# Improbable-AI/walk-these-ways

Hardware: AMD Instinct MI355X
Metric: env-steps/sec (sim+PPO) (higher is better)
Workload: dtype f32

## Files before the change

include/go1ppo.h:

```cpp
#ifndef GO1PPO_H
#define GO1PPO_H
#include <stdint.h>

#ifdef __cplusplus
extern "C" {
#endif

#define GO1PPO_ABI_VERSION 3
#define GO1PPO_MAX_ACTIONS 32

int go1ppo_elu_fwd(void* y, int64_t rows, int cols, int ld, const void* lat, int lat_ld, int npv, const void* wz,
                   int wz_ld, int lat_cols, void* stream);

int go1ppo_elu_bwd(const void* d, int ld_d, const void* h, int ld_h, int64_t rows, int cols, float* bias_grad, void* out,
                   int ld_out, void* stream);

typedef struct {
  const void* mean;
  const void* value;
  const float* std;
  int32_t head_ld, num_actions;
  int64_t rows;
  const int64_t* idx;
  const float* actions;
  const float* old_mu;
  const float* old_sigma;
  const float* old_logp;
  const float* advantages;
  const float* returns;
  const float* old_values;
  float clip_param, value_loss_coef, entropy_coef;
  int32_t use_clipped_value_loss;
  void* d_mean;
  void* d_value;
  float* d_std;
  float* d_mean_bias;
  float* d_value_bias;
  float* kl;
  float* value_loss;
  float* surrogate_loss;
} Go1PpoLossArgs;

int go1ppo_loss(const Go1PpoLossArgs* args, void* stream);

int go1ppo_mse(const void* pred, int pred_ld, const float* target, int npv, const int64_t* idx, int64_t rows,
               int64_t num_train, int selective, void* d_pred, float* d_pred_bias, float* train_loss,
               float* test_loss, void* stream);

int go1ppo_wgrad(const void* dz, int ld_dz, const void* h, int ld_h, int64_t rows, int n, int k, float* dW, int ldw,
                 float* bias_grad, void* stream);

#define GO1PPO_TAIL_MAX_LAYERS 4
#define GO1PPO_TAIL_MAX_NETS 3
typedef struct {
  const void* W;
  const void* bias;
  void* out;
  int32_t n_out, k_in, ld_out, elu;
} Go1PpoTailLayer;
typedef struct {
  const void* in;
  int64_t rows;
  int32_t ld_in, num_layers;
  int32_t elu_in, npv;
  const void* latent;
  const void* wz;
  int32_t lat_ld, wz_ld;
  Go1PpoTailLayer layer[GO1PPO_TAIL_MAX_LAYERS];
} Go1PpoTailNet;
typedef struct {
  int32_t num_nets, _pad;
  Go1PpoTailNet net[GO1PPO_TAIL_MAX_NETS];
} Go1PpoTailArgs;
int go1ppo_tail_fwd(const Go1PpoTailArgs* args, void* stream);

typedef struct {
  const void* dz;
  const void* h;
  float* dW;
  float* bias_grad;
  int64_t rows;
  int32_t ld_dz, ld_h, n, k, ldw;
  int32_t chunk_rows, wg_offset;
  int32_t zero_n, zero_k0, zero_k1;
  float* partials;
  int64_t partial_stride;
} Go1PpoWgradProblem;

int go1ppo_wgrad_plan(Go1PpoWgradProblem* host_problems, int count);
int go1ppo_wgrad_batched(const Go1PpoWgradProblem* device_problems, int count, int total_workgroups, void* stream);


int go1ppo_act(const void* mean, const void* value, int head_ld, const float* std, int num_actions, int64_t rows,
               const float* noise, float* actions, float* mu, float* sigma, float* values, float* logp, void* stream);

int go1ppo_store_step(const float* rewards, const uint8_t* dones, const uint8_t* time_outs, const int32_t* env_bins,
                      const float* values, float gamma, int64_t n, float* rewards_out, uint8_t* dones_out,
                      float* env_bins_out, void* stream);

int go1ppo_gae(const float* rewards, const uint8_t* dones, const float* values, const float* last_values, int T, int64_t N,
               float gamma, float lam, float* returns, float* advantages, double* stats, void* stream);

int go1ppo_normalize(float* adv, int64_t n, const double* stats, void* stream);


int go1ppo_ring_snapshot(const float* hist, int64_t ld_hist, int64_t N, int H, int no, void* ring, void* stream);

int go1ppo_ring_step(const float* obs, const float* priv, void* ring_dst, const void* ring_window, int64_t N, int H, int no,
                     int npv, int Kp, void* X, float* obs_store, float* priv_store, void* stream);

int go1ppo_ring_gather(const void* ring, const float* priv_store, const int64_t* idx, int64_t rows, int64_t N, int H, int no,
                       int npv, int Kp, void* X, void* stream);


int go1ppo_opt_partials(void);

int go1ppo_opt_prestep(const float* g, int64_t n, float gscale, float* partial, float* step, float* lr, const float* kl,
                       float kl_scale, float desired_kl, float lr_min, float lr_max, void* stream);

typedef struct {
  int64_t begin, count;
  const void* src;
  int64_t stride;
  int32_t kind, slabs, cols, zero_rows, zero_c0, zero_c1;
} Go1PpoGradPiece;
int go1ppo_grad_reduce(float* g, const Go1PpoGradPiece* device_pieces, int num_pieces, void* stream);
int go1ppo_opt_prestep_pieces(float* g, int64_t n, const Go1PpoGradPiece* device_pieces, int num_pieces, float gscale, float* partial,
                              float* step, float* lr, const float* kl, float kl_scale, float desired_kl, float lr_min, float lr_max,
                              void* stream);

#define GO1PPO_ADAM_MAX_TRANSPOSES 2
typedef struct {
  int32_t num_transposes, _pad;
  struct { int64_t start; int32_t rows, cols; void* dst; } transpose[GO1PPO_ADAM_MAX_TRANSPOSES];
} Go1PpoAdamExtras;
int go1ppo_opt_adam(float* p, float* g, float* m, float* v, int64_t start0, int64_t count0, int64_t start1,
                    int64_t count1, float gscale, const float* partial, float max_norm, const float* step, const float* lr,
                    float beta1, float beta2, float eps, void* body, int64_t n_body, float* tail, int64_t n_tail, int zero_grad,
                    float* zero_slot, const Go1PpoAdamExtras* extras, void* stream);

int go1ppo_sum_partials(const void* partials, int count, int64_t stride, int64_t rows, int cols, float* out, int zero_rows,
                        int zero_c0, int zero_c1, void* stream);


typedef struct Go1PpoGemmArgs {
  const void* A; const void* B; void* C; const float* bias; const void* H;
  int32_t M, N, K, lda, ldb, ldc, ldh, epilogue, elu_c0, elu_c1;
  int32_t elu_skip_c0, elu_skip_c1;
  int32_t bias_bf16, _pad;
} Go1PpoGemmArgs;
int go1ppo_gemm_nt(const Go1PpoGemmArgs* args, void* stream);
int go1ppo_gemm_nt_pair(const Go1PpoGemmArgs* a, const Go1PpoGemmArgs* b, void* stream);

int go1ppo_wgrad_tn_plan(Go1PpoWgradProblem* problems, int count);
int go1ppo_wgrad_tn_batched(const Go1PpoWgradProblem* device_problems, int count, int total_workgroups, void* stream);

#define GO1PPO_MLP2_MAX_NETS 3
typedef struct {
  void* x;
  const void* W2; const void* b2;
  const void* W3; const void* b3;
  void* z2;
  void* out;
  int64_t rows;
  int32_t ld_x, ld_z2, ld_out, elu_input;
} Go1PpoMlp2Fwd;
int go1ppo_mlp2_fwd(const Go1PpoMlp2Fwd* nets, int count, void* stream);

typedef struct {
  const void* d_out;
  const void* z2; const void* h;
  const void* W2; const void* W3;
  void* d_z2;
  void* d_x;
  int64_t rows;
  int32_t ld_dout, ld_z2, ld_h, ld_dz2, ld_dx, _pad;
} Go1PpoMlp2Bwd;
int go1ppo_mlp2_bwd(const Go1PpoMlp2Bwd* nets, int count, void* stream);

const char* go1ppo_version(void);

#ifdef __cplusplus
}
#endif
#endif
```

walk-these-ways_amd/csrc/go1ppo_mlp.h:

```cpp
#pragma once

#define MLP2_K1 256
#define MLP2_N2 128
#define MLP2_N3 64
#define MLP2_BM 64
#define MLP2_WAVES 16
#define MLP2_THREADS (64 * MLP2_WAVES)
#define MLP2_IMG (128 * 128)

struct Mlp2FwdArgs { Go1PpoMlp2Fwd net[GO1PPO_MLP2_MAX_NETS]; };
struct Mlp2BwdArgs { Go1PpoMlp2Bwd net[GO1PPO_MLP2_MAX_NETS]; };

__device__ __forceinline__ int swz_row(int row) { return row & 15; }
__device__ __forceinline__ int swz_red(int row) { return 2 * ((row & 3) | (((row >> 3) & 1) << 2)); }

template <bool RED>
__device__ __forceinline__ void dma_weights(const bf16_t* W, int rows, int cols, bf16_t* img, int wave, int lane) {
  const int windows = cols >> 7, count = (rows >> 2) * windows;
  for (int idx = wave; idx < count; idx += MLP2_WAVES) {
    const int win = idx % windows, blk = idx / windows;
    const int row = blk * 4 + (lane >> 4);
    const int chunk = (lane & 15) ^ (RED ? swz_red(row) : swz_row(row));
    glds16(W + (int64_t)row * cols + win * 128 + chunk * 8, img + win * MLP2_IMG + blk * 4 * 128);
  }
}

__device__ __forceinline__ uint2 pack_bf4(const float (&v)[4]) {
  f32x2 lo = {v[0], v[1]}, hi = {v[2], v[3]};
  uint2 o;
  o.x = __builtin_bit_cast(uint32_t, __builtin_convertvector(lo, bf16x2_t));
  o.y = __builtin_bit_cast(uint32_t, __builtin_convertvector(hi, bf16x2_t));
  return o;
}
__device__ __forceinline__ void unpack_bf4(uint2 r, float (&v)[4]) {
  v[0] = __uint_as_float(r.x << 16); v[1] = __uint_as_float(r.x & 0xffff0000u);
  v[2] = __uint_as_float(r.y << 16); v[3] = __uint_as_float(r.y & 0xffff0000u);
}
__device__ __forceinline__ bf16x8_t lds_b128(const bf16_t* img, int byte_off) {
  return *reinterpret_cast<const bf16x8_t*>(reinterpret_cast<const char*>(img) + byte_off);
}
__device__ __forceinline__ bf16x8_t lds_tr_operand(const bf16_t* img, int byte_off) {
  typedef __attribute__((address_space(3))) s16x4_t lds_s16x4_t;
  const char* p = reinterpret_cast<const char*>(img) + byte_off;
  s16x4_t lo = __builtin_amdgcn_ds_read_tr16_b64_v4i16((lds_s16x4_t*)(p));
  s16x4_t hi = __builtin_amdgcn_ds_read_tr16_b64_v4i16((lds_s16x4_t*)(p + 4 * 256));
  s16x8_t v = __builtin_shufflevector(lo, hi, 0, 1, 2, 3, 4, 5, 6, 7);
  return __builtin_bit_cast(bf16x8_t, v);
}

__global__ __launch_bounds__(MLP2_THREADS, 1) void mlp2_fwd_kernel(Mlp2FwdArgs A) {
  __shared__ __attribute__((aligned(1024))) bf16_t W2i[2 * MLP2_IMG];
  __shared__ __attribute__((aligned(1024))) bf16_t W3i[64 * 128];
  __shared__ __attribute__((aligned(1024))) bf16_t Ai[2 * 64 * 128];
  __shared__ __attribute__((aligned(1024))) bf16_t Z2i[64 * 128];
  const Go1PpoMlp2Fwd& N = A.net[blockIdx.y];
  const int tiles = (int)((N.rows + MLP2_BM - 1) / MLP2_BM);
  if ((int)blockIdx.x >= tiles) return;
  const int t = threadIdx.x, wave = t >> 6, lane = t & 63, r = lane & 15, g = lane >> 4;
  dma_weights<false>((const bf16_t*)N.W2, MLP2_N2, MLP2_K1, W2i, wave, lane);
  dma_weights<false>((const bf16_t*)N.W3, MLP2_N3, MLP2_N2, W3i, wave, lane);
  bf16_t* x = (bf16_t*)N.x;
  bf16_t* z2 = (bf16_t*)N.z2;
  bf16_t* out = (bf16_t*)N.out;
  const int tx = g ^ r;
  int foff[4];
#pragma unroll
  for (int a = 0; a < 4; a++) foff[a] = r * 256 + (((4 * a) ^ tx) << 4);
  const int nf2 = wave >> 1, mp = (wave & 1) * 2, nf3 = wave & 3, m3 = wave >> 2;
  float bias2[4], bias3[4];
  unpack_bf4(*reinterpret_cast<const uint2*>((const bf16_t*)N.b2 + nf2 * 16 + 4 * g), bias2);
  unpack_bf4(*reinterpret_cast<const uint2*>((const bf16_t*)N.b3 + nf3 * 16 + 4 * g), bias3);

  Bf8 v[2];
  auto fetch = [&](int tile) {
#pragma unroll
    for (int j = 0; j < 2; j++) {
      const int p = t + MLP2_THREADS * j, row = p >> 5, ch = p & 31;
      int64_t grow = (int64_t)tile * MLP2_BM + row;
      grow = grow < N.rows ? grow : N.rows - 1;
      v[j] = *reinterpret_cast<const Bf8*>(x + grow * N.ld_x + ch * 8);
    }
  };
  fetch(blockIdx.x);
  bool first = true;
  for (int tile = blockIdx.x; tile < tiles; tile += gridDim.x) {
    const int64_t row0 = (int64_t)tile * MLP2_BM;
#pragma unroll
    for (int j = 0; j < 2; j++) {
      const int p = t + MLP2_THREADS * j, row = p >> 5, ch = p & 31;
      if (N.elu_input) {
        float f[8];
#pragma unroll
        for (int e = 0; e < 8; e++) f[e] = elu1(bf2f(v[j].v[e]));
        v[j] = pack_bf8(f);
        if (row0 + row < N.rows) *reinterpret_cast<Bf8*>(x + (row0 + row) * N.ld_x + ch * 8) = v[j];
      }
      *reinterpret_cast<Bf8*>(reinterpret_cast<char*>(Ai + (ch >> 4) * 64 * 128) + row * 256 + (((ch & 15) ^ swz_row(row)) << 4)) = v[j];
    }
    if (first) asm volatile("s_waitcnt vmcnt(0)" ::: "memory");
    first = false;
    __syncthreads();
    if (tile + (int)gridDim.x < tiles) fetch(tile + gridDim.x);
    {
      f32x4 acc[2] = {f32x4{0.f, 0.f, 0.f, 0.f}, f32x4{0.f, 0.f, 0.f, 0.f}};
#pragma unroll
      for (int ks = 0; ks < MLP2_K1 / 32; ks++) {
        const int win = ks >> 2, off = foff[ks & 3];
        const bf16x8_t w = lds_b128(W2i + win * MLP2_IMG + nf2 * 16 * 128, off);
#pragma unroll
        for (int m = 0; m < 2; m++)
          acc[m] = __builtin_amdgcn_mfma_f32_16x16x32_bf16(w, lds_b128(Ai + win * 64 * 128 + (mp + m) * 16 * 128, off), acc[m], 0, 0, 0);
      }
      const int n0 = nf2 * 16 + 4 * g;
#pragma unroll
      for (int m = 0; m < 2; m++) {
        const int row = (mp + m) * 16 + r;
        float o4[4];
#pragma unroll
        for (int e = 0; e < 4; e++) o4[e] = elu1(acc[m][e] + bias2[e]);
        const uint2 o = pack_bf4(o4);
        if (row0 + row < N.rows) *reinterpret_cast<uint2*>(z2 + (row0 + row) * N.ld_z2 + n0) = o;
        *reinterpret_cast<uint2*>(reinterpret_cast<char*>(Z2i) + row * 256 + (((n0 >> 3) ^ swz_row(row)) << 4) + ((n0 >> 2) & 1) * 8) = o;
      }
    }
    __syncthreads();
    {
      f32x4 acc = f32x4{0.f, 0.f, 0.f, 0.f};
#pragma unroll
      for (int ks = 0; ks < MLP2_N2 / 32; ks++)
        acc = __builtin_amdgcn_mfma_f32_16x16x32_bf16(lds_b128(W3i + nf3 * 16 * 128, foff[ks]), lds_b128(Z2i + m3 * 16 * 128, foff[ks]), acc, 0, 0, 0);
      const int n0 = nf3 * 16 + 4 * g, row = m3 * 16 + r;
      float o4[4];
#pragma unroll
      for (int e = 0; e < 4; e++) o4[e] = acc[e] + bias3[e];
      if (row0 + row < N.rows) *reinterpret_cast<uint2*>(out + (row0 + row) * N.ld_out + n0) = pack_bf4(o4);
    }
  }
}

__global__ __launch_bounds__(MLP2_THREADS, 1) void mlp2_bwd_kernel(Mlp2BwdArgs A) {
  __shared__ __attribute__((aligned(1024))) bf16_t W3t[64 * 128];
  __shared__ __attribute__((aligned(1024))) bf16_t W2t[2 * MLP2_IMG];
  __shared__ __attribute__((aligned(1024))) bf16_t D3i[64 * 128];
  __shared__ __attribute__((aligned(1024))) bf16_t D2i[64 * 128];
  __shared__ __attribute__((aligned(1024))) bf16_t Hi[2 * 64 * 128];
  const Go1PpoMlp2Bwd& N = A.net[blockIdx.y];
  const int tiles = (int)((N.rows + MLP2_BM - 1) / MLP2_BM);
  if ((int)blockIdx.x >= tiles) return;
  const int t = threadIdx.x, wave = t >> 6, lane = t & 63, r = lane & 15, g = lane >> 4;
  dma_weights<true>((const bf16_t*)N.W3, MLP2_N3, MLP2_N2, W3t, wave, lane);
  dma_weights<true>((const bf16_t*)N.W2, MLP2_N2, MLP2_K1, W2t, wave, lane);
  const bf16_t* d = (const bf16_t*)N.d_out;
  const bf16_t* z2 = (const bf16_t*)N.z2;
  const bf16_t* hin = (const bf16_t*)N.h;
  bf16_t* dz2 = (bf16_t*)N.d_z2;
  bf16_t* dx = (bf16_t*)N.d_x;
  const int tx = g ^ r;
  int foff[4];
#pragma unroll
  for (int a = 0; a < 4; a++) foff[a] = r * 256 + (((4 * a) ^ tx) << 4);
  const int troff = (g * 8 + (r >> 2)) * 256 + ((r & 3) >> 1) * 16 + (r & 1) * 8;
  const int swb = 32 * ((r >> 2) | ((g & 1) << 2));
  const int kf2 = wave >> 1, mp = (wave & 1) * 2;
  const int w3off = troff + (((kf2 * 16) * 2) ^ swb);
  const bf16_t* w2img = W2t + (wave >> 3) * MLP2_IMG;
  const int w2off = troff + ((((wave & 7) * 16) * 2) ^ swb);
  const int hch = t & 31;
#define MLP2_HROW(j) ((t + (j) * MLP2_THREADS) >> 5)
  const int zrow = t >> 4, zch = t & 15, drow = (t >> 3) & 63, dch = t & 7;
#define MLP2_HSLOT(j) ((hch >> 4) * (64 * 128 * 2) + MLP2_HROW(j) * 256 + (((hch & 15) ^ swz_row(MLP2_HROW(j))) << 4))
  const int zslot = zrow * 256 + ((zch ^ swz_row(zrow)) << 4), dslot = drow * 256 + ((dch ^ swz_row(drow)) << 4);

  uint4 dv = make_uint4(0, 0, 0, 0), zv, hv0, hv1;
#define MLP2_BWD_FETCH(tile_)                                                                                          \
  {                                                                                                                    \
    const int64_t base = (int64_t)(tile_) * MLP2_BM, last = N.rows - 1;                                                \
    int64_t q = base + drow; q = q < last ? q : last;                                                                  \
    if (t < 512) dv = *reinterpret_cast<const uint4*>(d + q * N.ld_dout + dch * 8);                                      \
    q = base + zrow; q = q < last ? q : last;                                                                          \
    zv = *reinterpret_cast<const uint4*>(z2 + q * N.ld_z2 + zch * 8);                                                    \
    q = base + MLP2_HROW(0); q = q < last ? q : last;                                                                  \
    hv0 = *reinterpret_cast<const uint4*>(hin + q * N.ld_h + hch * 8);                                                   \
    q = base + MLP2_HROW(1); q = q < last ? q : last;                                                                  \
    hv1 = *reinterpret_cast<const uint4*>(hin + q * N.ld_h + hch * 8);                                                   \
  }
  MLP2_BWD_FETCH(blockIdx.x);
  bool first = true;
  for (int tile = blockIdx.x; tile < tiles; tile += gridDim.x) {
    const int64_t row0 = (int64_t)tile * MLP2_BM;
    if (t < 512) *reinterpret_cast<uint4*>(reinterpret_cast<char*>(D3i) + dslot) = dv;
    *reinterpret_cast<uint4*>(reinterpret_cast<char*>(D2i) + zslot) = zv;
    *reinterpret_cast<uint4*>(reinterpret_cast<char*>(Hi) + MLP2_HSLOT(0)) = hv0;
    *reinterpret_cast<uint4*>(reinterpret_cast<char*>(Hi) + MLP2_HSLOT(1)) = hv1;
    if (first) asm volatile("s_waitcnt vmcnt(0)" ::: "memory");
    first = false;
    __syncthreads();
    if (tile + (int)gridDim.x < tiles) MLP2_BWD_FETCH(tile + gridDim.x);
    {
      f32x4 acc[2] = {f32x4{0.f, 0.f, 0.f, 0.f}, f32x4{0.f, 0.f, 0.f, 0.f}};
#pragma unroll
      for (int kk = 0; kk < MLP2_N3 / 32; kk++) {
        const bf16x8_t w = lds_tr_operand(W3t, kk * 32 * 256 + w3off);
#pragma unroll
        for (int m = 0; m < 2; m++) acc[m] = __builtin_amdgcn_mfma_f32_16x16x32_bf16(w, lds_b128(D3i + (mp + m) * 16 * 128, foff[kk]), acc[m], 0, 0, 0);
      }
      const int k0 = kf2 * 16 + 4 * g;
#pragma unroll
      for (int m = 0; m < 2; m++) {
        const int row = (mp + m) * 16 + r;
        uint2* slot = reinterpret_cast<uint2*>(reinterpret_cast<char*>(D2i) + row * 256 + (((k0 >> 3) ^ swz_row(row)) << 4) + ((k0 >> 2) & 1) * 8);
        float h[4], o4[4];
        unpack_bf4(*slot, h);
#pragma unroll
        for (int e = 0; e < 4; e++) o4[e] = acc[m][e] * (h[e] > 0.f ? 1.f : h[e] + 1.f);
        *slot = pack_bf4(o4);
      }
    }
    __syncthreads();
    {
      f32x4 acc[4];
#pragma unroll
      for (int m = 0; m < 4; m++) acc[m] = f32x4{0.f, 0.f, 0.f, 0.f};
#pragma unroll
      for (int kk = 0; kk < MLP2_N2 / 32; kk++) {
        const bf16x8_t w = lds_tr_operand(w2img, kk * 32 * 256 + w2off);
#pragma unroll
        for (int m = 0; m < 4; m++) acc[m] = __builtin_amdgcn_mfma_f32_16x16x32_bf16(w, lds_b128(D2i + m * 16 * 128, foff[kk]), acc[m], 0, 0, 0);
      }
      const int k0 = (wave & 7) * 16 + 4 * g;
#pragma unroll
      for (int m = 0; m < 4; m++) {
        const int row = m * 16 + r;
        uint2* slot = reinterpret_cast<uint2*>(reinterpret_cast<char*>(Hi + (wave >> 3) * 64 * 128) + row * 256 +
                                               (((k0 >> 3) ^ swz_row(row)) << 4) + ((k0 >> 2) & 1) * 8);
        float h[4], o4[4];
        unpack_bf4(*slot, h);
#pragma unroll
        for (int e = 0; e < 4; e++) o4[e] = acc[m][e] * (h[e] > 0.f ? 1.f : h[e] + 1.f);
        *slot = pack_bf4(o4);
      }
    }
    __syncthreads();
    if (row0 + zrow < N.rows) put16_wt(dz2 + (row0 + zrow) * N.ld_dz2 + zch * 8, *reinterpret_cast<const uint4*>(reinterpret_cast<const char*>(D2i) + zslot));
#pragma unroll
    for (int j = 0; j < 2; j++)
      if (row0 + MLP2_HROW(j) < N.rows)
        put16_wt(dx + (row0 + MLP2_HROW(j)) * N.ld_dx + hch * 8, *reinterpret_cast<const uint4*>(reinterpret_cast<const char*>(Hi) + MLP2_HSLOT(j)));
    __syncthreads();
  }
}

static inline bool aligned8(const void* p) { return (reinterpret_cast<uintptr_t>(p) & 7) == 0; }

extern "C" int go1ppo_mlp2_fwd(const Go1PpoMlp2Fwd* nets, int count, void* stream) {
  if (!nets || count <= 0 || count > GO1PPO_MLP2_MAX_NETS) return -1;
  Mlp2FwdArgs A;
  int64_t max_rows = 0;
  for (int i = 0; i < count; i++) {
    const Go1PpoMlp2Fwd& N = nets[i];
    if (!N.x || !N.W2 || !N.b2 || !N.W3 || !N.b3 || !N.z2 || !N.out || N.rows <= 0) return -1;
    if ((N.ld_x & 7) || (N.ld_z2 & 3) || (N.ld_out & 3) || N.ld_x < MLP2_K1 || N.ld_z2 < MLP2_N2 || N.ld_out < MLP2_N3 || !aligned16(N.x) ||
        !aligned16(N.W2) || !aligned16(N.W3) || !aligned8(N.b2) || !aligned8(N.b3) || !aligned8(N.z2) || !aligned8(N.out))
      return -2;
    A.net[i] = N;
    if (N.rows > max_rows) max_rows = N.rows;
  }
  int64_t wgs = (max_rows + MLP2_BM - 1) / MLP2_BM;
  if (wgs > 256 / count) wgs = 256 / count;
  mlp2_fwd_kernel<<<dim3((unsigned)wgs, count), dim3(MLP2_THREADS), 0, (hipStream_t)stream>>>(A);
  return hipGetLastError() == hipSuccess ? 0 : -9;
}

extern "C" int go1ppo_mlp2_bwd(const Go1PpoMlp2Bwd* nets, int count, void* stream) {
  if (!nets || count <= 0 || count > GO1PPO_MLP2_MAX_NETS) return -1;
  Mlp2BwdArgs A;
  int64_t max_rows = 0;
  for (int i = 0; i < count; i++) {
    const Go1PpoMlp2Bwd& N = nets[i];
    if (!N.d_out || !N.z2 || !N.h || !N.W2 || !N.W3 || !N.d_z2 || !N.d_x || N.rows <= 0) return -1;
    if ((N.ld_dout & 7) || (N.ld_z2 & 7) || (N.ld_h & 7) || (N.ld_dz2 & 7) || (N.ld_dx & 7) || N.ld_dout < MLP2_N3 || N.ld_z2 < MLP2_N2 ||
        N.ld_h < MLP2_K1 || N.ld_dz2 < MLP2_N2 || N.ld_dx < MLP2_K1 || !aligned16(N.d_out) || !aligned16(N.W2) || !aligned16(N.W3) ||
        !aligned16(N.z2) || !aligned16(N.h) || !aligned16(N.d_z2) || !aligned16(N.d_x))
      return -2;
    A.net[i] = N;
    if (N.rows > max_rows) max_rows = N.rows;
  }
  int64_t wgs = (max_rows + MLP2_BM - 1) / MLP2_BM;
  if (wgs > 256 / count) wgs = 256 / count;
  mlp2_bwd_kernel<<<dim3((unsigned)wgs, count), dim3(MLP2_THREADS), 0, (hipStream_t)stream>>>(A);
  return hipGetLastError() == hipSuccess ? 0 : -9;
}
```

walk-these-ways_amd/go1_gym_learn/ppo_cse/fused.py:

```python
import ctypes
import os

import torch

HEAD = 64
_HERE = os.path.dirname(os.path.abspath(__file__))
_LIB_PATH = os.path.normpath(os.path.join(_HERE, "..", "..", "csrc", "libgo1ppo.so"))
_lib = None


class Go1PpoLibraryMissing(RuntimeError):
    pass


class LossArgs(ctypes.Structure):
    _fields_ = [("mean", ctypes.c_void_p), ("value", ctypes.c_void_p), ("std", ctypes.c_void_p),
                ("head_ld", ctypes.c_int32), ("num_actions", ctypes.c_int32), ("rows", ctypes.c_int64),
                ("idx", ctypes.c_void_p), ("actions", ctypes.c_void_p), ("old_mu", ctypes.c_void_p),
                ("old_sigma", ctypes.c_void_p), ("old_logp", ctypes.c_void_p), ("advantages", ctypes.c_void_p),
                ("returns", ctypes.c_void_p), ("old_values", ctypes.c_void_p),
                ("clip_param", ctypes.c_float), ("value_loss_coef", ctypes.c_float), ("entropy_coef", ctypes.c_float),
                ("use_clipped_value_loss", ctypes.c_int32),
                ("d_mean", ctypes.c_void_p), ("d_value", ctypes.c_void_p), ("d_std", ctypes.c_void_p),
                ("d_mean_bias", ctypes.c_void_p), ("d_value_bias", ctypes.c_void_p), ("kl", ctypes.c_void_p),
                ("value_loss", ctypes.c_void_p), ("surrogate_loss", ctypes.c_void_p)]


class WgradProblem(ctypes.Structure):
    _fields_ = [("dz", ctypes.c_void_p), ("h", ctypes.c_void_p), ("dW", ctypes.c_void_p), ("bias_grad", ctypes.c_void_p),
                ("rows", ctypes.c_int64), ("ld_dz", ctypes.c_int32), ("ld_h", ctypes.c_int32), ("n", ctypes.c_int32),
                ("k", ctypes.c_int32), ("ldw", ctypes.c_int32), ("chunk_rows", ctypes.c_int32), ("wg_offset", ctypes.c_int32),
                ("zero_n", ctypes.c_int32), ("zero_k0", ctypes.c_int32), ("zero_k1", ctypes.c_int32),
                ("partials", ctypes.c_void_p), ("partial_stride", ctypes.c_int64)]


class GradPiece(ctypes.Structure):
    _fields_ = [("begin", ctypes.c_int64), ("count", ctypes.c_int64), ("src", ctypes.c_void_p), ("stride", ctypes.c_int64),
                ("kind", ctypes.c_int32), ("slabs", ctypes.c_int32), ("cols", ctypes.c_int32), ("zero_rows", ctypes.c_int32),
                ("zero_c0", ctypes.c_int32), ("zero_c1", ctypes.c_int32)]


class TailLayer(ctypes.Structure):
    _fields_ = [("W", ctypes.c_void_p), ("bias", ctypes.c_void_p), ("out", ctypes.c_void_p), ("n_out", ctypes.c_int32),
                ("k_in", ctypes.c_int32), ("ld_out", ctypes.c_int32), ("elu", ctypes.c_int32)]


class TailNet(ctypes.Structure):
    _fields_ = [("in_", ctypes.c_void_p), ("rows", ctypes.c_int64), ("ld_in", ctypes.c_int32), ("num_layers", ctypes.c_int32),
                ("elu_in", ctypes.c_int32), ("npv", ctypes.c_int32), ("latent", ctypes.c_void_p), ("wz", ctypes.c_void_p),
                ("lat_ld", ctypes.c_int32), ("wz_ld", ctypes.c_int32),
                ("layer", TailLayer * 4)]


class TailArgs(ctypes.Structure):
    _fields_ = [("num_nets", ctypes.c_int32), ("_pad", ctypes.c_int32), ("net", TailNet * 3)]


class Mlp2Fwd(ctypes.Structure):
    _fields_ = [(n, ctypes.c_void_p) for n in ("x", "W2", "b2", "W3", "b3", "z2", "out")] + [("rows", ctypes.c_int64)] + \
               [(n, ctypes.c_int32) for n in ("ld_x", "ld_z2", "ld_out", "elu_input")]


class Mlp2Bwd(ctypes.Structure):
    _fields_ = [(n, ctypes.c_void_p) for n in ("d_out", "z2", "h", "W2", "W3", "d_z2", "d_x")] + [("rows", ctypes.c_int64)] + \
               [(n, ctypes.c_int32) for n in ("ld_dout", "ld_z2", "ld_h", "ld_dz2", "ld_dx", "_pad")]


MLP2_DIMS = (256, 128, 64)


class GemmArgs(ctypes.Structure):
    _fields_ = [("A", ctypes.c_void_p), ("B", ctypes.c_void_p), ("C", ctypes.c_void_p), ("bias", ctypes.c_void_p),
                ("H", ctypes.c_void_p)] + [(n, ctypes.c_int32) for n in
                                           ("M", "N", "K", "lda", "ldb", "ldc", "ldh", "epilogue", "elu_c0", "elu_c1", "elu_skip_c0", "elu_skip_c1", "bias_bf16", "_pad")]


class _AdamTranspose(ctypes.Structure):
    _fields_ = [("start", ctypes.c_int64), ("rows", ctypes.c_int32), ("cols", ctypes.c_int32), ("dst", ctypes.c_void_p)]


class AdamExtras(ctypes.Structure):
    _fields_ = [("num_transposes", ctypes.c_int32), ("_pad", ctypes.c_int32), ("transpose", _AdamTranspose * 2)]


EXPORTED_SYMBOLS = ["go1ppo_mlp2_fwd", "go1ppo_mlp2_bwd", "go1ppo_gemm_nt", "go1ppo_gemm_nt_pair", "go1ppo_sum_partials", "go1ppo_wgrad_tn_plan", "go1ppo_wgrad_tn_batched", "go1ppo_tail_fwd", "go1ppo_elu_fwd", "go1ppo_elu_bwd", "go1ppo_loss", "go1ppo_mse", "go1ppo_wgrad", "go1ppo_wgrad_plan",
                    "go1ppo_wgrad_batched", "go1ppo_act",
                    "go1ppo_store_step", "go1ppo_ring_snapshot", "go1ppo_ring_step", "go1ppo_ring_gather", "go1ppo_gae", "go1ppo_normalize", "go1ppo_opt_partials", "go1ppo_opt_prestep",
                    "go1ppo_opt_prestep_pieces", "go1ppo_grad_reduce", "go1ppo_opt_adam", "go1ppo_version"]


def load_library(path=None):
    global _lib
    if _lib is not None and path is None:
        return _lib
    p = path or _LIB_PATH
    if not os.path.exists(p):
        raise Go1PpoLibraryMissing(f"{p} not found: run `python -c 'import __graft_entry__ as g; g.build()'` "
                                   "(hipcc --offload-arch=gfx950); the fused PPO update has no CPU fallback")
    L = ctypes.CDLL(p)
    vp, i32, i64 = ctypes.c_void_p, ctypes.c_int, ctypes.c_int64
    L.go1ppo_elu_fwd.argtypes = [vp, i64, i32, i32, vp, i32, i32, vp, i32, i32, vp]
    L.go1ppo_elu_bwd.argtypes = [vp, i32, vp, i32, i64, i32, vp, vp, i32, vp]
    L.go1ppo_loss.argtypes = [ctypes.POINTER(LossArgs), vp]
    L.go1ppo_mse.argtypes = [vp, i32, vp, i32, vp, i64, i64, i32, vp, vp, vp, vp, vp]
    L.go1ppo_wgrad.argtypes = [vp, i32, vp, i32, i64, i32, i32, vp, i32, vp, vp]
    L.go1ppo_wgrad_plan.argtypes = [ctypes.POINTER(WgradProblem), i32]
    L.go1ppo_tail_fwd.argtypes = [ctypes.POINTER(TailArgs), vp]
    L.go1ppo_gemm_nt.argtypes = [ctypes.POINTER(GemmArgs), vp]
    L.go1ppo_gemm_nt_pair.argtypes = [ctypes.POINTER(GemmArgs), ctypes.POINTER(GemmArgs), vp]
    L.go1ppo_sum_partials.argtypes = [vp, i32, i64, i64, i32, vp, i32, i32, i32, vp]
    L.go1ppo_mlp2_fwd.argtypes = [ctypes.POINTER(Mlp2Fwd), i32, vp]
    L.go1ppo_mlp2_bwd.argtypes = [ctypes.POINTER(Mlp2Bwd), i32, vp]
    L.go1ppo_wgrad_batched.argtypes = [vp, i32, i32, vp]
    L.go1ppo_wgrad_tn_plan.argtypes = [ctypes.POINTER(WgradProblem), i32]
    L.go1ppo_wgrad_tn_batched.argtypes = [vp, i32, i32, vp]
    f32 = ctypes.c_float
    L.go1ppo_act.argtypes = [vp, vp, i32, vp, i32, i64, vp, vp, vp, vp, vp, vp, vp]
    L.go1ppo_store_step.argtypes = [vp, vp, vp, vp, vp, f32, i64, vp, vp, vp, vp]
    L.go1ppo_ring_snapshot.argtypes = [vp, i64, i64, i32, i32, vp, vp]
    L.go1ppo_ring_step.argtypes = [vp, vp, vp, vp, i64, i32, i32, i32, i32, vp, vp, vp, vp]
    L.go1ppo_ring_gather.argtypes = [vp, vp, vp, i64, i64, i32, i32, i32, i32, vp, vp]
    L.go1ppo_gae.argtypes = [vp, vp, vp, vp, i32, i64, f32, f32, vp, vp, vp, vp]
    L.go1ppo_normalize.argtypes = [vp, i64, vp, vp]
    L.go1ppo_opt_partials.argtypes = []
    L.go1ppo_opt_prestep.argtypes = [vp, i64, f32, vp, vp, vp, vp, f32, f32, f32, f32, vp]
    L.go1ppo_opt_prestep_pieces.argtypes = [vp, i64, vp, i32, f32, vp, vp, vp, vp, f32, f32, f32, f32, vp]
    L.go1ppo_grad_reduce.argtypes = [vp, vp, i32, vp]
    L.go1ppo_opt_adam.argtypes = [vp, vp, vp, vp, i64, i64, i64, i64, f32, vp, f32, vp, vp, f32, f32, f32, vp, i64, vp, i64, i32, vp,
                                  ctypes.POINTER(AdamExtras), vp]
    for name in EXPORTED_SYMBOLS[:-1]:
        getattr(L, name).restype = ctypes.c_int
    L.go1ppo_version.restype = ctypes.c_char_p
    if path is None:
        _lib = L
    return L


def _stream():
    return torch.cuda.current_stream().cuda_stream


def _chk(rc, what):
    if rc != 0:
        raise RuntimeError(f"{what} failed with code {rc}")


def _ptr(t):
    return None if t is None else t.data_ptr()


def _ld(t):
    assert t.dim() == 2 and t.stride(1) == 1
    return t.stride(0)


def gemm_args(a, b, c, bias=None, elu=None, elu_bwd_of=None, elu_skip=None):
    g = GemmArgs()
    g.A, g.B, g.C, g.bias, g.H = a.data_ptr(), b.data_ptr(), c.data_ptr(), _ptr(bias), _ptr(elu_bwd_of)
    g.M, g.N, g.K, g.lda, g.ldb, g.ldc = a.shape[0], b.shape[0], a.shape[1], _ld(a), _ld(b), _ld(c)
    assert b.shape[1] == g.K and tuple(c.shape) == (g.M, g.N) and (elu is None or elu_bwd_of is None)
    assert a.dtype == b.dtype == c.dtype == torch.bfloat16 and (bias is None or bias.dtype in (torch.float32, torch.bfloat16))
    g.bias_bf16 = int(bias is not None and bias.dtype == torch.bfloat16)
    if elu_bwd_of is not None:
        assert elu_bwd_of.shape == c.shape and elu_bwd_of.dtype == torch.bfloat16
        g.epilogue, g.ldh = 2, _ld(elu_bwd_of)
    elif elu is not None:
        g.epilogue = 1
        g.elu_c0, g.elu_c1 = (0, g.N) if elu is True else elu
        if elu_skip is not None:
            g.elu_skip_c0, g.elu_skip_c1 = elu_skip
    return g


def gemm_nt(lib, a, b, c, bias=None, elu=None, elu_bwd_of=None):
    g = gemm_args(a, b, c, bias, elu, elu_bwd_of)
    _chk(lib.go1ppo_gemm_nt(ctypes.byref(g), _stream()), "go1ppo_gemm_nt")
    return c


def gemm_nt_pair(lib, first, second):
    ga, gb = gemm_args(**first), gemm_args(**second)
    _chk(lib.go1ppo_gemm_nt_pair(ctypes.byref(ga), ctypes.byref(gb), _stream()), "go1ppo_gemm_nt_pair")


class FusedNet:

    def __init__(self, policy, body, grad, M, lib, with_grad, two_streams=True, fused_tails=None):
        assert body.dtype == torch.bfloat16 and body.is_cuda
        self.pol, self.M, self.lib = policy, M, lib
        dev = body.device
        self.P = {name: policy._block(body, name) for name, _ in policy.blocks}
        self.G = {name: policy._block(grad, name) for name, _ in policy.blocks} if grad is not None else None
        self.nd, self.na, self.nc = policy.first
        self.n1 = self.nd + self.na + self.nc
        self.depth = {n: len(l) for n, l in policy.nets.items()}
        bf = dict(device=dev, dtype=torch.bfloat16)
        self.Y1 = torch.zeros(M, self.n1, **bf)
        self.Y1d = torch.zeros(M, self.nd, **bf)
        self.Z = {n: {li: torch.zeros(M, self.P[f"{n}.{li}.W"].shape[0], **bf) for li in range(1, d)}
                  for n, d in self.depth.items()}
        assert policy.npv <= HEAD and self.P["Wz"].shape == (self.na, HEAD)
        self._recording, self._batched, self._plans = None, False, {}
        self._grad = grad
        self.defer_grad_sum = False
        self._rec_pieces, self._slab_ws, self._last_pieces = None, {}, {}
        self._wgrad_tn = M % 64 == 0
        self._tails = self._tails_ad = None
        if fused_tails is None:
            fused_tails = M <= int(os.environ.get("GO1_FUSED_TAILS_MAX_ROWS", "2048"))
        self._elu_on_load = not with_grad
        if fused_tails and self._fused_tails_ok():
            nd, na = self.nd, self.na
            eol = self._elu_on_load
            self._tails = (self._tail_args([("adaptation", self.Y1[:, :nd])], with_grad, elu_in=eol),
                           self._tail_args([("actor", self.Y1[:, nd:nd + na]), ("critic", self.Y1[:, nd + na:])], with_grad, elu_in=eol,
                                           latent_for="actor" if eol else None))
            self._tails_ad = self._tail_args([("adaptation", self.Y1d)], with_grad)
        self._mlp2 = (self._tails is None and os.environ.get("GO1_MLP2", "1") == "1" and self.nd == MLP2_DIMS[0] and
                      all(self.depth[n] >= 3 and tuple(self.P[f"{n}.{self.depth[n] - 2}.W"].shape) == (MLP2_DIMS[1], MLP2_DIMS[0])
                          and tuple(self.P[f"{n}.{self.depth[n] - 1}.W"].shape) == (MLP2_DIMS[2], MLP2_DIMS[1]) for n in self.depth)
                      and self.depth["adaptation"] == 3 and self.depth["actor"] == 4 and self.depth["critic"] == 4)
        self._mlp2_cache = {}
        na1, nc1 = int(self.P["actor.1.W"].shape[0]), int(self.P["critic.1.W"].shape[0])
        nt_ok = all(v % 64 == 0 for v in (na1, nc1, self.na, self.n1 - self.nd - self.na)) and \
            all(self.P[k].data_ptr() % 16 == 0 for k in ("actor.1.b", "critic.1.b", "actor.1.W", "critic.1.W"))
        pair_ok = nt_ok and na1 == nc1 and self.na == self.n1 - self.nd - self.na
        self._l1_nt = nt_ok
        self._pair = pair_ok
        self._side = torch.cuda.Stream(device=dev) if two_streams else None
        if with_grad:
            self.X = torch.zeros(M, policy.Kp, **bf)
            self.dH1 = {"adaptation": torch.zeros(M, self.nd, **bf), "actor": torch.zeros(M, self.na, **bf),
                        "critic": torch.zeros(M, self.nc, **bf)}
            self.dY1 = torch.zeros(M, self.n1, **bf)
            self.dZ = {n: {li: torch.zeros_like(z) for li, z in zs.items()} for n, zs in self.Z.items()}
            w1_split = next((b for b in (M // 6144, 4, 2) if b >= 2 and M % b == 0 and (M // b) % 64 == 0), 1)
            self._w1_tmp = torch.zeros(w1_split, self.n1, policy.Kp, **bf)
            self._dgrad_nt = self._mlp2 and nt_ok
            self._WT = {n: torch.zeros(self.P[f"{n}.1.W"].shape[1], self.P[f"{n}.1.W"].shape[0], **bf) for n in ("actor", "critic")} \
                if self._dgrad_nt else None
            self._wt_by_optimizer = False
            self.priv_mask = (self.nd + self.na, policy.K + 1, policy.K + 1 + policy.npv)

    def _elu(self, y, lat=None, lat_cols=0):
        wz = self.P["Wz"] if lat is not None else None
        _chk(self.lib.go1ppo_elu_fwd(y.data_ptr(), y.shape[0], y.shape[1], _ld(y), _ptr(lat), _ld(lat) if lat is not None else 0,
                                     self.pol.npv if lat is not None else 0, _ptr(wz), HEAD, lat_cols, _stream()), "go1ppo_elu_fwd")

    def _elu_bwd(self, d, h, bias_grad, out=None):
        out = d if out is None else out
        _chk(self.lib.go1ppo_elu_bwd(d.data_ptr(), _ld(d), _ptr(h), _ld(h) if h is not None else 0, d.shape[0], d.shape[1],
                                     _ptr(bias_grad), out.data_ptr(), _ld(out), _stream()), "go1ppo_elu_bwd")

    def _wgrad(self, dz, h, gW, gb=None, zero=None):
        n, k = dz.shape[1], h.shape[1]
        assert gW.shape == (n, k) and gW.is_contiguous()
        if self._recording is not None:
            self._recording.append((dz, h, gW, gb, zero))
            return
        if self._batched:
            return
        assert zero is None or zero[0] == 0, "the structural zeros are applied by the batched launch"
        _chk(self.lib.go1ppo_wgrad(dz.data_ptr(), _ld(dz), h.data_ptr(), _ld(h), dz.shape[0], n, k, gW.data_ptr(), k, _ptr(gb),
                                   _stream()), "go1ppo_wgrad")

    def _tail_args(self, nets_and_inputs, keep_intermediates, elu_in=False, latent_for=None):
        a = TailArgs()
        a.num_nets = len(nets_and_inputs)
        for N, (net, h) in zip(a.net, nets_and_inputs):
            d = self.depth[net]
            N.in_, N.rows, N.ld_in, N.num_layers = h.data_ptr(), h.shape[0], _ld(h), d - 1
            N.elu_in = int(bool(elu_in))
            if elu_in and latent_for == net:
                lat, wz = self.Z["adaptation"][self.depth["adaptation"] - 1], self.P["Wz"]
                N.latent, N.wz, N.lat_ld, N.wz_ld, N.npv = lat.data_ptr(), wz.data_ptr(), _ld(lat), HEAD, self.pol.npv
            for li in range(1, d):
                L, W, z = N.layer[li - 1], self.P[f"{net}.{li}.W"], self.Z[net][li]
                last = li == d - 1
                L.W, L.bias = W.data_ptr(), self.P[f"{net}.{li}.b"].data_ptr()
                L.out = z.data_ptr() if (last or keep_intermediates) else None
                L.n_out, L.k_in, L.ld_out, L.elu = W.shape[0], W.shape[1], _ld(z), 0 if last else 1
        return a

    def _fused_tails_ok(self):
        ok = all(self.depth[n] - 1 <= 4 for n in self.depth)
        for n, d in self.depth.items():
            for li in range(1, d):
                r, k = self.P[f"{n}.{li}.W"].shape
                ok = ok and k % 32 == 0 and k <= 512 and r % 16 == 0 and r <= 512
        return ok

    def _tail(self, net, h):
        P, d = self.P, self.depth[net]
        for li in range(1, d):
            z = self.Z[net][li]
            torch.addmm(P[f"{net}.{li}.b"], h, P[f"{net}.{li}.W"].t(), out=z)
            if li < d - 1:
                self._elu(z)
            h = z
        return h

    def forward(self, x):
        nd, na = self.nd, self.na
        if self._mlp2:
            return self._forward_mlp2(x)
        torch.mm(x, self.P["W1"].t(), out=self.Y1)
        if self._tails is not None:
            ta, tac = self._tails
            if not self._elu_on_load:
                self._elu(self.Y1[:, :nd])
            _chk(self.lib.go1ppo_tail_fwd(ctypes.byref(ta), _stream()), "go1ppo_tail_fwd")
            latent = self.Z["adaptation"][self.depth["adaptation"] - 1]
            if not self._elu_on_load:
                self._elu(self.Y1[:, nd:], latent, na)
            _chk(self.lib.go1ppo_tail_fwd(ctypes.byref(tac), _stream()), "go1ppo_tail_fwd")
            return self.Z["actor"][self.depth["actor"] - 1], self.Z["critic"][self.depth["critic"] - 1], latent
        self._elu(self.Y1[:, :nd])
        latent = self._tail("adaptation", self.Y1[:, :nd])
        self._elu(self.Y1[:, nd:], latent, na)
        with self._branch():
            value = self._tail("critic", self.Y1[:, nd + na:])
        mean = self._tail("actor", self.Y1[:, nd:nd + na])
        self._join()
        return mean, value, latent

    def _mlp2_fwd(self, key, items, elu_input=1):
        key = ("fwd", key, elu_input)
        if key not in self._mlp2_cache:
            arr = (Mlp2Fwd * len(items))()
            for a, (net, x) in zip(arr, items):
                d = self.depth[net]
                W2, W3, z2, out = self.P[f"{net}.{d - 2}.W"], self.P[f"{net}.{d - 1}.W"], self.Z[net][d - 2], self.Z[net][d - 1]
                a.x, a.W2, a.b2, a.W3, a.b3 = x.data_ptr(), W2.data_ptr(), self.P[f"{net}.{d - 2}.b"].data_ptr(), W3.data_ptr(), self.P[f"{net}.{d - 1}.b"].data_ptr()
                a.z2, a.out, a.rows, a.ld_x, a.ld_z2, a.ld_out, a.elu_input = z2.data_ptr(), out.data_ptr(), x.shape[0], _ld(x), _ld(z2), _ld(out), int(elu_input)
            self._mlp2_cache[key] = (arr, len(items))
        arr, n = self._mlp2_cache[key]
        _chk(self.lib.go1ppo_mlp2_fwd(arr, n, _stream()), "go1ppo_mlp2_fwd")

    def _mlp2_bwd(self, key, items):
        key = ("bwd", key)
        if key not in self._mlp2_cache:
            arr = (Mlp2Bwd * len(items))()
            for a, (net, h, d_x) in zip(arr, items):
                d = self.depth[net]
                d_out, z2, d_z2 = self.dZ[net][d - 1], self.Z[net][d - 2], self.dZ[net][d - 2]
                a.d_out, a.z2, a.h, a.W2, a.W3 = d_out.data_ptr(), z2.data_ptr(), h.data_ptr(), self.P[f"{net}.{d - 2}.W"].data_ptr(), self.P[f"{net}.{d - 1}.W"].data_ptr()
                a.d_z2, a.d_x, a.rows = d_z2.data_ptr(), d_x.data_ptr(), h.shape[0]
                a.ld_dout, a.ld_z2, a.ld_h, a.ld_dz2, a.ld_dx = _ld(d_out), _ld(z2), _ld(h), _ld(d_z2), _ld(d_x)
            self._mlp2_cache[key] = (arr, len(items))
        arr, n = self._mlp2_cache[key]
        _chk(self.lib.go1ppo_mlp2_bwd(arr, n, _stream()), "go1ppo_mlp2_bwd")

    def _forward_mlp2(self, x):
        P, Z, nd, na = self.P, self.Z, self.nd, self.na
        torch.mm(x, P["W1"].t(), out=self.Y1)
        self._mlp2_fwd("adaptation", [("adaptation", self.Y1[:, :nd])])
        latent = Z["adaptation"][2]
        self._elu(self.Y1[:, nd:], latent, na)
        if self._l1_nt and self._pair:
            gemm_nt_pair(self.lib, dict(a=self.Y1[:, nd:nd + na], b=P["actor.1.W"], c=Z["actor"][1], bias=P["actor.1.b"]),
                         dict(a=self.Y1[:, nd + na:], b=P["critic.1.W"], c=Z["critic"][1], bias=P["critic.1.b"]))
        elif self._l1_nt:
            with self._branch():
                gemm_nt(self.lib, self.Y1[:, nd + na:], P["critic.1.W"], Z["critic"][1], P["critic.1.b"])
            gemm_nt(self.lib, self.Y1[:, nd:nd + na], P["actor.1.W"], Z["actor"][1], P["actor.1.b"])
        else:
            with self._branch():
                torch.addmm(P["critic.1.b"], self.Y1[:, nd + na:], P["critic.1.W"].t(), out=Z["critic"][1])
            torch.addmm(P["actor.1.b"], self.Y1[:, nd:nd + na], P["actor.1.W"].t(), out=Z["actor"][1])
        self._join()
        self._mlp2_fwd("ac", [("actor", Z["actor"][1]), ("critic", Z["critic"][1])])
        return Z["actor"][3], Z["critic"][3], latent

    def _backward_mlp2(self, x):
        nd, na = self.nd, self.na
        P, G, Z, dZ, Y1, dY1, dH1 = self.P, self.G, self.Z, self.dZ, self.Y1, self.dY1, self.dH1
        cols = {"adaptation": slice(0, nd), "actor": slice(nd, nd + na), "critic": slice(nd + na, self.n1)}
        self._mlp2_bwd("ac", [("actor", Z["actor"][1], dZ["actor"][1]), ("critic", Z["critic"][1], dZ["critic"][1])])
        for net in ("actor", "critic"):
            self._wgrad(dZ[net][3], Z[net][2], G[f"{net}.3.W"], None)
            self._wgrad(dZ[net][2], Z[net][1], G[f"{net}.2.W"], G[f"{net}.2.b"])
            self._wgrad(dZ[net][1], Y1[:, cols[net]], G[f"{net}.1.W"], G[f"{net}.1.b"])
        if self._dgrad_nt and self._pair and self._wt_by_optimizer:
            gemm_nt_pair(self.lib, dict(a=dZ["actor"][1], b=self._WT["actor"], c=dY1[:, cols["actor"]], elu_bwd_of=Y1[:, cols["actor"]]),
                         dict(a=dZ["critic"][1], b=self._WT["critic"], c=dY1[:, cols["critic"]], elu_bwd_of=Y1[:, cols["critic"]]))
        elif self._dgrad_nt:
            with self._branch():
                if not self._wt_by_optimizer:
                    self._WT["critic"].copy_(P["critic.1.W"].t())
                gemm_nt(self.lib, dZ["critic"][1], self._WT["critic"], dY1[:, cols["critic"]], elu_bwd_of=Y1[:, cols["critic"]])
            if not self._wt_by_optimizer:
                self._WT["actor"].copy_(P["actor.1.W"].t())
            gemm_nt(self.lib, dZ["actor"][1], self._WT["actor"], dY1[:, cols["actor"]], elu_bwd_of=Y1[:, cols["actor"]])
        else:
            with self._branch():
                torch.mm(dZ["critic"][1], P["critic.1.W"], out=dH1["critic"])
                self._elu_bwd(dH1["critic"], Y1[:, cols["critic"]], None, out=dY1[:, cols["critic"]])
            torch.mm(dZ["actor"][1], P["actor.1.W"], out=dH1["actor"])
            self._elu_bwd(dH1["actor"], Y1[:, cols["actor"]], None, out=dY1[:, cols["actor"]])
        latent, dlat = Z["adaptation"][2], dZ["adaptation"][2]
        dA1 = dY1[:, cols["actor"]]
        self._wgrad(dA1, latent, G["Wz"])
        torch.mm(dA1, P["Wz"], out=dlat)
        self._mlp2_bwd("adaptation", [("adaptation", Y1[:, :nd], dY1[:, :nd])])
        self._wgrad(dlat, Z["adaptation"][1], G["adaptation.2.W"], G["adaptation.2.b"])
        self._wgrad(dZ["adaptation"][1], Y1[:, :nd], G["adaptation.1.W"], G["adaptation.1.b"])
        self._join()
        self._big_wgrad(dY1, x, G["W1"], self._w1_tmp)

    def _forward_adaptation_mlp2(self, x):
        torch.mm(x, self.P["W1"][:self.nd].t(), out=self.Y1d)
        self._mlp2_fwd("adaptation_only", [("adaptation", self.Y1d)])
        return self.Z["adaptation"][2]

    def _backward_adaptation_mlp2(self, x):
        nd, d, G, Z, dZ = self.nd, self.dH1["adaptation"], self.G, self.Z, self.dZ
        self._mlp2_bwd("adaptation_only", [("adaptation", self.Y1d, d)])
        self._wgrad(dZ["adaptation"][2], Z["adaptation"][1], G["adaptation.2.W"], None)
        self._wgrad(dZ["adaptation"][1], self.Y1d, G["adaptation.1.W"], G["adaptation.1.b"])
        self._big_wgrad(d, x, G["W1"][:nd], self._w1_tmp[:, :nd], own_kernel=self._wgrad_tn)

    def adam_transposes(self):
        if not getattr(self, "_dgrad_nt", False):
            return []
        out = []
        for n in ("actor", "critic"):
            i = self.pol.index[f"{n}.1.W"]
            rows, cols = self.pol.blocks[i][1]
            out.append((self.pol.offsets[i], rows, cols, self._WT[n]))
        return out

    def refresh_transposes(self):
        if getattr(self, "_dgrad_nt", False):
            for n in ("actor", "critic"):
                self._WT[n].copy_(self.P[f"{n}.1.W"].t())

    def _branch(self):
        if self._side is None:
            import contextlib
            return contextlib.nullcontext()
        self._side.wait_stream(torch.cuda.current_stream())
        self._forked = True
        return torch.cuda.stream(self._side)

    def _join(self):
        if self._side is not None and getattr(self, "_forked", False):
            torch.cuda.current_stream().wait_stream(self._side)
            self._forked = False

    def forward_adaptation(self, x):
        if self._mlp2:
            return self._forward_adaptation_mlp2(x)
        torch.mm(x, self.P["W1"][:self.nd].t(), out=self.Y1d)
        self._elu(self.Y1d)
        if self._tails_ad is not None:
            _chk(self.lib.go1ppo_tail_fwd(ctypes.byref(self._tails_ad), _stream()), "go1ppo_tail_fwd")
            return self.Z["adaptation"][self.depth["adaptation"] - 1]
        return self._tail("adaptation", self.Y1d)

    def _tail_bwd(self, net, h0, dh0, head_bias_done=True):
        P, G, d = self.P, self.G, self.depth[net]
        for li in range(d - 1, 0, -1):
            dz = self.dZ[net][li]
            h_in = self.Z[net][li - 1] if li > 1 else h0
            gb = None if (li == d - 1 and head_bias_done) else G[f"{net}.{li}.b"]
            self._wgrad(dz, h_in, G[f"{net}.{li}.W"], gb)
            out = self.dZ[net][li - 1] if li > 1 else dh0
            torch.mm(dz, P[f"{net}.{li}.W"], out=out)
            if li > 1:
                self._elu_bwd(out, h_in, None)

    def _big_wgrad(self, dY, x, gW, tmp, own_kernel=False):
        zr, zc0, zc1 = self.priv_mask
        zr = min(zr, gW.shape[0])
        if own_kernel:
            self._wgrad(dY, x, gW, zero=(zr, zc0, zc1))
            return
        b = tmp.shape[0]
        if b == 1 or not tmp.is_contiguous():
            torch.mm(dY.t(), x, out=tmp[0])
            part, count, stride = tmp[0], 1, gW.numel()
        else:
            torch.bmm(dY.view(b, dY.shape[0] // b, dY.shape[1]).transpose(1, 2), x.view(b, x.shape[0] // b, x.shape[1]), out=tmp)
            part, count, stride = tmp, b, tmp.stride(0)
        assert gW.is_contiguous() and part.stride(-1) == 1 and part.stride(-2) == gW.shape[1]
        if self._rec_pieces is not None:
            self._rec_pieces.append(dict(begin=self._grad_offset(gW), count=gW.numel(), src=part, stride=stride, kind=2, slabs=count,
                                         cols=gW.shape[1], zero=(zr, zc0, zc1)))

    def _grad_offset(self, view):
        off = (view.data_ptr() - self._grad.data_ptr()) // 4
        assert view.dtype == torch.float32 and view.is_contiguous() and 0 <= off and off + view.numel() <= self._grad.numel()
        return int(off)

    def last_pieces(self, kind):
        return self._last_pieces.get(kind)

    def _run_planned(self, key, fn):
        if key not in self._plans:
            self._recording, self._rec_pieces = [], []
            fn()
            rec, self._recording = self._recording, None
            pieces, self._rec_pieces = self._rec_pieces, None
            tab = (WgradProblem * len(rec))()
            for P, (dz, h, gW, gb, zero) in zip(tab, rec):
                P.dz, P.h, P.dW, P.bias_grad = dz.data_ptr(), h.data_ptr(), gW.data_ptr(), _ptr(gb)
                if zero is not None:
                    P.zero_n, P.zero_k0, P.zero_k1 = zero
                P.rows, P.ld_dz, P.ld_h, P.n, P.k, P.ldw = dz.shape[0], _ld(dz), _ld(h), dz.shape[1], h.shape[1], gW.shape[1]
            tn = self._wgrad_tn and all(P.rows % 64 == 0 and P.n % 8 == 0 and P.k % 8 == 0 for P in tab)
            plan = self.lib.go1ppo_wgrad_tn_plan if tn else self.lib.go1ppo_wgrad_plan
            if tn:
                for P, (dz, h, gW, gb, zero) in zip(tab, rec):
                    P.partials, P.partial_stride = 16, gW.numel()
            total = plan(tab, len(rec))
            if total <= 0:
                raise RuntimeError(f"go1ppo_wgrad_plan failed with code {total}")
            if tn:
                for j, (P, (dz, h, gW, gb, zero)) in enumerate(zip(tab, rec)):
                    S = -(-P.rows // P.chunk_rows)
                    ws = self._slab_ws.get((key[0], j))
                    if ws is None or tuple(ws.shape) != (S, gW.numel()):
                        ws = self._slab_ws[(key[0], j)] = torch.zeros(S, gW.numel(), device=gW.device, dtype=torch.float32)
                    P.partials, P.partial_stride = ws.data_ptr(), gW.numel()
                    pieces.append(dict(begin=self._grad_offset(gW), count=gW.numel(), src=ws, stride=gW.numel(), kind=1, slabs=S, cols=gW.shape[1],
                                       zero=(0, 0, 0)))
                if plan(tab, len(rec)) != total:
                    raise RuntimeError("go1ppo_wgrad_tn_plan: the plan changed with the slab buffers attached")
            dev = torch.frombuffer(bytearray(bytes(tab)), dtype=torch.uint8).to(self.Y1.device)
            ptab = None
            if pieces:
                pieces.sort(key=lambda q: q["begin"])
                arr = (GradPiece * len(pieces))()
                end = 0
                for A, q in zip(arr, pieces):
                    assert q["begin"] >= end and q["begin"] % 8 == 0 and q["count"] % 8 == 0 and q["stride"] % 8 == 0, "slab pieces: ascending, disjoint, multiples of 8"
                    end = q["begin"] + q["count"]
                    A.begin, A.count, A.src, A.stride, A.kind, A.slabs, A.cols = q["begin"], q["count"], q["src"].data_ptr(), q["stride"], q["kind"], q["slabs"], q["cols"]
                    A.zero_rows, A.zero_c0, A.zero_c1 = q["zero"]
                ptab = (torch.frombuffer(bytearray(bytes(arr)), dtype=torch.uint8).to(self.Y1.device), len(pieces), [q["src"] for q in pieces])
            self._plans[key] = (dev, len(rec), total, rec, tn, ptab)
        else:
            self._batched = True
            try:
                fn()
            finally:
                self._batched = False
        dev, count, total, _, tn, ptab = self._plans[key]
        launch = self.lib.go1ppo_wgrad_tn_batched if tn else self.lib.go1ppo_wgrad_batched
        _chk(launch(dev.data_ptr(), count, total, _stream()), "go1ppo_wgrad_batched")
        self._last_pieces[key[0]] = None
        if ptab is None:
            return
        if self.defer_grad_sum:
            self._last_pieces[key[0]] = ptab[:2]
        else:
            _chk(self.lib.go1ppo_grad_reduce(self._grad.data_ptr(), ptab[0].data_ptr(), ptab[1], _stream()), "go1ppo_grad_reduce")

    def backward(self, x):
        self._run_planned(("ppo", x.data_ptr()), lambda: (self._backward_mlp2 if self._mlp2 else self._backward)(x))

    def backward_adaptation(self, x):
        self._run_planned(("adaptation", x.data_ptr()), lambda: (self._backward_adaptation_mlp2 if self._mlp2 else self._backward_adaptation)(x))

    def _backward(self, x):
        nd, na = self.nd, self.na
        G, Y1, dY1, dH1 = self.G, self.Y1, self.dY1, self.dH1
        cols = {"adaptation": slice(0, nd), "actor": slice(nd, nd + na), "critic": slice(nd + na, self.n1)}
        with self._branch():
            self._tail_bwd("critic", Y1[:, cols["critic"]], dH1["critic"])
            self._elu_bwd(dH1["critic"], Y1[:, cols["critic"]], None, out=dY1[:, cols["critic"]])
        self._tail_bwd("actor", Y1[:, cols["actor"]], dH1["actor"])
        self._elu_bwd(dH1["actor"], Y1[:, cols["actor"]], None, out=dY1[:, cols["actor"]])
        last = self.depth["adaptation"] - 1
        latent, dlat = self.Z["adaptation"][last], self.dZ["adaptation"][last]
        dA1 = dY1[:, cols["actor"]]
        self._wgrad(dA1, latent, G["Wz"])
        torch.mm(dA1, self.P["Wz"], out=dlat)
        self._tail_bwd("adaptation", Y1[:, :nd], dH1["adaptation"], head_bias_done=False)
        self._elu_bwd(dH1["adaptation"], Y1[:, :nd], None, out=dY1[:, :nd])
        self._join()
        self._big_wgrad(dY1, x, G["W1"], self._w1_tmp)

    def _backward_adaptation(self, x):
        nd, d = self.nd, self.dH1["adaptation"]
        self._tail_bwd("adaptation", self.Y1d, d)
        self._elu_bwd(d, self.Y1d, None)
        self._big_wgrad(d, x, self.G["W1"][:nd], self._w1_tmp[:, :nd], own_kernel=self._wgrad_tn)

    def ppo_loss(self, st, idx, std, g_std, A, kl, acc):
        la, lc = self.depth["actor"] - 1, self.depth["critic"] - 1
        flat = lambda t: t.flatten(0, 1)
        a = LossArgs()
        a.mean, a.value, a.std = self.Z["actor"][la].data_ptr(), self.Z["critic"][lc].data_ptr(), std.data_ptr()
        a.head_ld, a.num_actions, a.rows = HEAD, std.numel(), self.M
        a.idx = idx.data_ptr()
        for field, t in (("actions", st.actions), ("old_mu", st.mu), ("old_sigma", st.sigma), ("old_logp", st.actions_log_prob),
                         ("advantages", st.advantages), ("returns", st.returns), ("old_values", st.values)):
            t = flat(t)
            assert t.is_contiguous() and t.dtype == torch.float32
            setattr(a, field, t.data_ptr())
        a.clip_param, a.value_loss_coef, a.entropy_coef = A.clip_param, A.value_loss_coef, A.entropy_coef
        a.use_clipped_value_loss = int(A.use_clipped_value_loss)
        a.d_mean, a.d_value = self.dZ["actor"][la].data_ptr(), self.dZ["critic"][lc].data_ptr()
        a.d_std = g_std.data_ptr()
        a.d_mean_bias = self.G[f"actor.{la}.b"].data_ptr()
        a.d_value_bias = self.G[f"critic.{lc}.b"].data_ptr()
        a.kl = kl.data_ptr()
        a.value_loss = acc[0:].data_ptr()
        a.surrogate_loss = acc[1:].data_ptr()
        _chk(self.lib.go1ppo_loss(ctypes.byref(a), _stream()), "go1ppo_loss")

    def adaptation_loss(self, st, idx, num_train, selective, acc):
        last = self.depth["adaptation"] - 1
        pred, dpred = self.Z["adaptation"][last], self.dZ["adaptation"][last]
        target = st.privileged_observations.flatten(0, 1)
        assert target.is_contiguous() and target.dtype == torch.float32 and target.shape[1] == self.pol.npv
        _chk(self.lib.go1ppo_mse(pred.data_ptr(), HEAD, target.data_ptr(), self.pol.npv, idx.data_ptr(), self.M, num_train,
                                 int(selective), dpred.data_ptr(), self.G[f"adaptation.{last}.b"].data_ptr(),
                                 acc[2:].data_ptr(), acc[3:].data_ptr(), _stream()), "go1ppo_mse")


def act(lib, mean, value, std, noise, st, s):
    _chk(lib.go1ppo_act(mean.data_ptr(), value.data_ptr(), _ld(mean), std.data_ptr(), std.numel(), mean.shape[0], noise.data_ptr(),
                        st.actions[s].data_ptr(), st.mu[s].data_ptr(), st.sigma[s].data_ptr(), st.values[s].data_ptr(),
                        st.actions_log_prob[s].data_ptr(), _stream()), "go1ppo_act")


def store_step(lib, st, s, rewards, dones, time_outs, env_bins, gamma):
    n = rewards.shape[0]
    for t, dt in ((rewards, torch.float32), (dones, torch.uint8)):
        assert t.is_contiguous() and t.dtype == dt and t.shape[0] == n
    if time_outs is not None:
        assert time_outs.is_contiguous() and time_outs.element_size() == 1
    if env_bins is not None:
        assert env_bins.is_contiguous() and env_bins.dtype == torch.int32
    _chk(lib.go1ppo_store_step(rewards.data_ptr(), dones.data_ptr(), _ptr(time_outs), _ptr(env_bins), st.values[s].data_ptr(), gamma, n,
                               st.rewards[s].data_ptr(), st.dones[s].data_ptr(), st.env_bins[s].data_ptr() if env_bins is not None else None,
                               _stream()), "go1ppo_store_step")


def ring_step(lib, st, s, obs, privileged_obs, obs_history, X):
    N, no, H = st.num_envs, st.obs_ring.shape[2], st.history_length
    npv = st.privileged_observations.shape[-1]
    for t in (obs, privileged_obs):
        assert t.dtype == torch.float32 and t.is_contiguous() and t.shape[0] == N
    assert X.dtype == torch.bfloat16 and X.is_contiguous() and tuple(X.shape) == (N, st.padded_width)
    if s == 0:
        assert obs_history.dtype == torch.float32 and obs_history.stride(1) == 1 and tuple(obs_history.shape) == (N, H * no)
        _chk(lib.go1ppo_ring_snapshot(obs_history.data_ptr(), obs_history.stride(0), N, H, no, st.obs_ring.data_ptr(), _stream()),
             "go1ppo_ring_snapshot")
    dst = None if s == 0 else st.obs_ring[s + H - 1].data_ptr()
    _chk(lib.go1ppo_ring_step(obs.data_ptr(), privileged_obs.data_ptr(), dst, st.obs_ring[s].data_ptr(), N, H, no, npv, st.padded_width,
                              X.data_ptr(), st.observations[s].data_ptr(), st.privileged_observations[s].data_ptr(), _stream()),
         "go1ppo_ring_step")


def ring_gather(lib, st, idx, X):
    N, no, H = st.num_envs, st.obs_ring.shape[2], st.history_length
    priv = st.privileged_observations
    assert idx.dtype == torch.int64 and idx.is_contiguous() and X.is_contiguous() and tuple(X.shape) == (idx.numel(), st.padded_width)
    assert priv.dtype == torch.float32 and priv.is_contiguous()
    _chk(lib.go1ppo_ring_gather(st.obs_ring.data_ptr(), priv.data_ptr(), idx.data_ptr(), idx.numel(), N, H, no, priv.shape[-1],
                                st.padded_width, X.data_ptr(), _stream()), "go1ppo_ring_gather")


def gae(lib, st, last_values, gamma, lam, stats):
    T, N = st.num_transitions_per_env, st.num_envs
    stats.zero_()
    _chk(lib.go1ppo_gae(st.rewards.data_ptr(), st.dones.data_ptr(), st.values.data_ptr(), last_values.data_ptr(), T, N, gamma, lam,
                        st.returns.data_ptr(), st.advantages.data_ptr(), stats.data_ptr(), _stream()), "go1ppo_gae")
    stats[2] = float(T * N)


def normalize(lib, st, stats):
    _chk(lib.go1ppo_normalize(st.advantages.data_ptr(), st.advantages.numel(), stats.data_ptr(), _stream()), "go1ppo_normalize")


class FusedAdam:

    def __init__(self, lib, master, body, std, n_body, lr, ranges=None, betas=(0.9, 0.999), eps=1e-8):
        self.lib, self.master, self.body, self.std, self.n_body = lib, master, body, std, n_body
        dev = master.device
        self.m, self.v = torch.zeros_like(master), torch.zeros_like(master)
        self.step = torch.zeros(1, device=dev)
        self.lr = torch.full((1,), float(lr), device=dev)
        self.partial = torch.zeros(lib.go1ppo_opt_partials(), device=dev)
        self.betas, self.eps = betas, eps
        r = list(ranges or [(0, master.numel())]) + [(0, 0)]
        self.r0, self.r1 = r[0], r[1]
        self.n_norm = max(a + b for a, b in r)
        self.extras = AdamExtras()
        self._keep = []

    def set_transposes(self, items):
        e = self.extras
        assert len(items) <= 2
        e.num_transposes = len(items)
        self._keep = [t for *_, t in items]
        for T, (start, rows, cols, dst) in zip(e.transpose, items):
            assert dst.is_contiguous() and dst.dtype == torch.bfloat16 and tuple(dst.shape) == (cols, rows)
            T.start, T.rows, T.cols, T.dst = int(start), int(rows), int(cols), dst.data_ptr()

    def set_ranges(self, ranges):
        r = list(ranges) + [(0, 0)]
        self.r0, self.r1 = r[0], r[1]

    def step_(self, gscale=1.0, max_norm=None, kl=None, kl_scale=1.0, desired_kl=0.01, lr_min=1e-5, lr_max=1e-2, zero_grad=False,
              zero_slot=None, between=None, pieces=None):
        g = self.master.grad
        clip = max_norm is not None
        if pieces is not None:
            _chk(self.lib.go1ppo_opt_prestep_pieces(g.data_ptr(), self.n_norm, pieces[0].data_ptr(), pieces[1], gscale, self.partial.data_ptr(),
                                                    self.step.data_ptr(), self.lr.data_ptr(), _ptr(kl), kl_scale, desired_kl, lr_min, lr_max,
                                                    _stream()), "go1ppo_opt_prestep_pieces")
        else:
            _chk(self.lib.go1ppo_opt_prestep(g.data_ptr(), self.n_norm, gscale, self.partial.data_ptr() if clip else None,
                                             self.step.data_ptr(), self.lr.data_ptr(), _ptr(kl), kl_scale, desired_kl, lr_min, lr_max,
                                             _stream()), "go1ppo_opt_prestep")
        if between is not None:
            between(self.partial)
        _chk(self.lib.go1ppo_opt_adam(self.master.data_ptr(), g.data_ptr(), self.m.data_ptr(), self.v.data_ptr(), self.r0[0], self.r0[1],
                                      self.r1[0], self.r1[1], gscale, self.partial.data_ptr() if clip else None,
                                      float(max_norm) if clip else 0.0, self.step.data_ptr(), self.lr.data_ptr(), self.betas[0],
                                      self.betas[1], self.eps, self.body.data_ptr(), self.n_body, self.std.data_ptr(), self.std.numel(), int(zero_grad),
                                      _ptr(zero_slot), ctypes.byref(self.extras), _stream()),
             "go1ppo_opt_adam")
```

walk-these-ways_amd/go1_gym_learn/ppo_cse/ppo.py:

```python
import math
import os
import sys

import torch
import torch.distributed as dist
import torch.nn.functional as F
import torch.optim as optim
from params_proto import PrefixProto

from go1_gym_learn.ppo_cse import ActorCritic
from go1_gym_learn.ppo_cse import RolloutStorage
from go1_gym_learn.ppo_cse import caches
from go1_gym_learn.ppo_cse.flat_policy import FlatPolicy


class PPO_Args(PrefixProto):
    value_loss_coef = 1.0
    use_clipped_value_loss = True
    clip_param = 0.2
    entropy_coef = 0.01
    num_learning_epochs = 5
    num_mini_batches = 4
    learning_rate = 1.e-3
    adaptation_module_learning_rate = 1.e-3
    num_adaptation_module_substeps = 1
    schedule = 'adaptive'
    gamma = 0.99
    lam = 0.95
    desired_kl = 0.01
    max_grad_norm = 1.
    selective_adaptation_module_loss = False
    autocast_bf16 = False
    data_parallel = True
    dp_grad_dtype = "fp32"
    dp_zero1 = False
    history_ring = True
    use_hip_graphs = True
    dp_graph_collectives = True
    use_fused_kernels = True
    use_tuned_gemms = True


_HALF_LOG_2PI = 0.5 * math.log(2.0 * math.pi)


def _enable_tuned_gemms():
    import os
    if "PYTORCH_TUNABLEOP_ENABLED" in os.environ:
        return
    try:
        from torch.cuda import tunable
        path = os.path.join(os.path.dirname(os.path.abspath(__file__)), "..", "..", "tuning", "tunableop_gfx950.csv")
        tunable.enable(True)
        tunable.set_filename(os.path.normpath(path), insert_device_ordinal=False)
        tunable.set_max_tuning_duration(30)
        if hasattr(tunable, "write_file_on_exit"):
            tunable.write_file_on_exit(False)
    except Exception as err:
        print(f"[ppo] TunableOp not enabled ({type(err).__name__}: {err})", file=sys.stderr)


_AUTOCAST_DEFAULT = bool(PPO_Args.autocast_bf16)


def policy_dtype_is_bf16():
    v = os.environ.get("GO1_POLICY_DTYPE", "").strip().lower()
    if v and v not in ("bf16", "bfloat16", "fp32", "f32", "float32"):
        raise ValueError(f"GO1_POLICY_DTYPE={v!r}: expected bf16 or fp32")
    if v:
        want = v in ("bf16", "bfloat16")
        explicit = bool(PPO_Args.autocast_bf16) != _AUTOCAST_DEFAULT
        if explicit and bool(PPO_Args.autocast_bf16) != want:
            raise ValueError(f"GO1_POLICY_DTYPE={v} contradicts PPO_Args.autocast_bf16={PPO_Args.autocast_bf16}")
        return want
    return bool(PPO_Args.autocast_bf16)


def _force_dp():
    return os.environ.get("GO1_FORCE_DP", "0") not in ("", "0")


def _world():
    return dist.get_world_size() if dist.is_available() and dist.is_initialized() else 1


def gaussian_log_prob(actions, mean, std):
    z = (actions - mean) / std
    return -0.5 * (z * z).sum(dim=-1) - (torch.log(std).sum() + actions.shape[-1] * _HALF_LOG_2PI)


def gaussian_entropy(std):
    return (0.5 + _HALF_LOG_2PI) * std.numel() + torch.log(std).sum()


class PPO:
    actor_critic: ActorCritic

    def __init__(self, actor_critic, device='cpu'):
        self.device = device
        self.actor_critic = actor_critic
        self.actor_critic.to(device)
        self.on_gpu = torch.device(device).type == "cuda"
        self.bf16 = bool(policy_dtype_is_bf16() and self.on_gpu)
        self.storage = None
        ac = self.actor_critic
        self.policy = FlatPolicy(ac)
        n = self.policy.numel
        self.n_body, self.n_std = n, ac.std.numel()
        w = _world() if PPO_Args.data_parallel else 1
        self.master = torch.zeros(-(-(n + 16) // w) * w, device=device)
        self.policy.pack(ac, self.master[:n])
        self.master[n:n + self.n_std].copy_(ac.std.detach())
        self.master.grad = torch.zeros_like(self.master)
        self._kl = self.master.grad[n + self.n_std:n + self.n_std + 1].view(())
        self._g_live = self.master.grad[:n + self.n_std]
        pol = self.policy
        self._priv_cols_grad = pol._block(self.master.grad[:n], "W1")[:pol.first[0] + pol.first[1], pol.K + 1:pol.K + 1 + pol.npv]
        self.body = torch.zeros(n, device=device, dtype=torch.bfloat16 if self.bf16 else torch.float32).requires_grad_()
        self.std = torch.zeros(self.n_std, device=device).requires_grad_()
        kw = dict(fused=True, capturable=True) if self.on_gpu else {}
        self._acc = torch.zeros(4, device=device)
        self._idx_all, self._graphs, self._updates_done = None, {}, 0
        self._collectives_capturable = None
        self._pregathered, self._Xall = False, None
        lr = torch.tensor(PPO_Args.learning_rate, device=device) if self.on_gpu else PPO_Args.learning_rate
        self.optimizer = optim.Adam([self.master], lr=lr, **kw)
        self.adaptation_module_optimizer = optim.Adam([self.master], lr=PPO_Args.adaptation_module_learning_rate, **kw)
        self.transition = RolloutStorage.Transition()
        self._lr = torch.tensor(PPO_Args.learning_rate, device=device)
        self.dp = bool(PPO_Args.data_parallel and (_world() > 1 or (_force_dp() and dist.is_available() and dist.is_initialized())))
        self.fused = bool(self.bf16 and PPO_Args.use_fused_kernels and self.policy.act is torch.nn.ELU)
        self._roll_net = self._train_net = None
        self._roll_noise = None
        self._update_graph_ok = True
        self._opt = self._opt_ad = None
        if self.on_gpu and PPO_Args.use_tuned_gemms:
            _enable_tuned_gemms()
        self._ad_grad_views = [self.master.grad]
        if self.fused:
            from go1_gym_learn.ppo_cse import fused
            self._fused_lib = fused.load_library()
            pol, ns = self.policy, self.n_std
            self._opt = fused.FusedAdam(self._fused_lib, self.master, self.body, self.std, n, PPO_Args.learning_rate, ranges=[(0, n + ns)])
            self._opt_ad = fused.FusedAdam(self._fused_lib, self.master, self.body, self.std, n, PPO_Args.adaptation_module_learning_rate,
                                           ranges=[(0, pol.adaptation_numel)])
            self._lr = self._opt.lr
            self._ad_grad_views = [self.master.grad[:pol.adaptation_numel]]
        if self.dp:
            dist.broadcast(self.master, src=0)
        self._dp_lowp = self._dp_shard = None
        if self.dp:
            A = PPO_Args
            assert A.dp_grad_dtype in ("fp32", "bf16")
            if A.dp_grad_dtype == "bf16":
                self._dp_lowp = torch.zeros(self.master.numel(), device=device, dtype=torch.bfloat16)
            if A.dp_zero1:
                per = self.master.numel() // _world()
                self._dp_shard = (dist.get_rank() * per, per)
                self._dp_shard_buf = torch.zeros(per, device=device, dtype=torch.bfloat16 if self._dp_lowp is not None else torch.float32)
                self._dp_tail = torch.zeros(self.master.numel() - n, device=device)
                if self._opt is not None:
                    lo = self._dp_shard[0]
                    self._opt.set_ranges([(lo, max(0, min(lo + per, n + self.n_std) - lo))])
        self._push_weights()

    @property
    def flat_param(self):
        return self.master

    @property
    def flat_grad(self):
        return self.master.grad

    def _push_weights(self):
        with torch.no_grad():
            self.body.copy_(self.master[:self.n_body])
            self.std.copy_(self.master[self.n_body:self.n_body + self.n_std])
            if self._train_net is not None:
                self._train_net.refresh_transposes()

    def _pull_grads(self):
        g = self.master.grad
        if self.body.grad is not None:
            g[:self.n_body].copy_(self.body.grad)
        else:
            g[:self.n_body].zero_()
        if self.std.grad is not None:
            g[self.n_body:self.n_body + self.n_std].copy_(self.std.grad)
        else:
            g[self.n_body:].zero_()
        self.body.grad = None
        self.std.grad = None
        self._priv_cols_grad.zero_()

    def sync_module(self):
        self.policy.unpack(self.master[:self.n_body], self.actor_critic)
        with torch.no_grad():
            self.actor_critic.std.copy_(self.master[self.n_body:self.n_body + self.n_std])
        return self.actor_critic

    def load_module(self):
        self.policy.pack(self.actor_critic, self.master[:self.n_body])
        with torch.no_grad():
            self.master[self.n_body:self.n_body + self.n_std].copy_(self.actor_critic.std)
        self._push_weights()

    @property
    def learning_rate(self):
        return float(self._lr)

    def init_storage(self, num_envs, num_transitions_per_env, actor_obs_shape, privileged_obs_shape, obs_history_shape,
                     action_shape, sliding_history=False):
        no = int(actor_obs_shape[0])
        ring = bool(sliding_history and self.fused and PPO_Args.history_ring and no % 2 == 0 and int(obs_history_shape[0]) % no == 0)
        self.storage = RolloutStorage(num_envs, num_transitions_per_env, actor_obs_shape, privileged_obs_shape,
                                      obs_history_shape, action_shape, self.device,
                                      history_dtype=self.body.dtype, history_pad_to=64, augment=True, ring=ring)
        assert self.storage.padded_width == self.policy.Kp
        self._last_hist = torch.zeros(num_envs, self.policy.Kp, device=self.device, dtype=self.body.dtype)
        self._last_hist[:, self.storage.history_width] = 1.0
        self._X_roll = torch.zeros_like(self._last_hist) if ring else None
        if self.fused:
            from go1_gym_learn.ppo_cse.fused import FusedNet
            self._roll_net = FusedNet(self.policy, self.body, None, num_envs, self._fused_lib, with_grad=False, two_streams=False)

    def test_mode(self):
        self.actor_critic.test()

    def train_mode(self):
        self.actor_critic.train()

    def act(self, obs, privileged_obs, obs_history):
        t = self.transition
        if self.storage.ring:
            return self._act_ring(obs, privileged_obs, obs_history)
        slot = self.storage.observation_histories[self.storage.step]
        self.storage.write_history(slot, obs_history, privileged_obs)
        t.observation_histories = slot
        if self._roll_net is not None and slot.shape[0] == self._roll_net.M:
            return self._act_fused(slot, obs, privileged_obs)
        mean, value = self._infer(slot)
        std = self.std.detach()
        t.actions = mean + std * torch.randn_like(mean)
        t.values = value.detach()
        t.actions_log_prob = gaussian_log_prob(t.actions, mean, std)
        t.action_mean = mean
        t.action_sigma = std.expand_as(mean)
        self._snapshot_obs(obs, privileged_obs)
        return t.actions

    def _snapshot_obs(self, obs, privileged_obs):
        t, st = self.transition, self.storage
        s = st.step
        if s >= st.num_transitions_per_env:
            raise AssertionError("Rollout buffer overflow")
        st.observations[s].copy_(obs)
        st.privileged_observations[s].copy_(privileged_obs)
        t.observations = t.critic_observations = st.observations[s]
        t.privileged_observations = st.privileged_observations[s]

    def _act_ring(self, obs, privileged_obs, obs_history):
        from go1_gym_learn.ppo_cse import fused
        st = self.storage
        s = st.step
        if s >= st.num_transitions_per_env:
            raise AssertionError("Rollout buffer overflow")
        if st.num_envs != self._roll_net.M:
            raise AssertionError("ring storage needs the static-buffer inference engine of its own batch size")
        fused.ring_step(self._fused_lib, st, s, obs.contiguous(), privileged_obs.contiguous(), obs_history, self._X_roll)
        self.transition.observation_histories = self._X_roll
        return self._act_fused(self._X_roll, obs, privileged_obs, stored=True)

    def _act_fused(self, slot, obs, privileged_obs, stored=False):
        from go1_gym_learn.ppo_cse import fused
        t, st = self.transition, self.storage
        s = st.step
        if s >= st.num_transitions_per_env:
            raise AssertionError("Rollout buffer overflow")
        with torch.no_grad():
            mean, value, _ = self._roll_net.forward(slot)
            T = st.num_transitions_per_env
            if s == 0 or self._roll_noise is None or tuple(self._roll_noise.shape) != (T, slot.shape[0], self.n_std):
                self._roll_noise = torch.randn(T, slot.shape[0], self.n_std, device=slot.device)
            noise = self._roll_noise[s]
            fused.act(self._fused_lib, mean, value, self.std, noise, st, s)
        t.actions, t.values, t.actions_log_prob = st.actions[s], st.values[s], st.actions_log_prob[s]
        t.action_mean, t.action_sigma = st.mu[s], st.sigma[s]
        if stored:
            t.observations = t.critic_observations = st.observations[s]
            t.privileged_observations = st.privileged_observations[s]
        else:
            self._snapshot_obs(obs, privileged_obs)
        return t.actions

    def _infer(self, rows):
        with torch.no_grad():
            if self._roll_net is not None and rows.shape[0] == self._roll_net.M:
                mean, value, _ = self._roll_net.forward(rows)
                return mean[:, :self.n_std].float(), value[:, :1].float()
            mean, value, _ = self.policy.forward(self.body, rows)
            return mean.float(), value.float()

    def process_env_step(self, rewards, dones, infos):
        t = self.transition
        if t.actions is not None and self._roll_net is not None and t.actions.data_ptr() == self.storage.actions[self.storage.step].data_ptr():
            return self._process_env_step_fused(rewards, dones, infos)
        t.rewards = rewards.clone()
        t.dones = dones
        t.env_bins = infos["env_bins"]
        if 'time_outs' in infos:
            t.rewards += PPO_Args.gamma * torch.squeeze(t.values * infos['time_outs'].unsqueeze(1).to(self.device), 1)
        self.storage.add_transitions(t)
        t.clear()
        self.actor_critic.reset(dones)

    def _process_env_step_fused(self, rewards, dones, infos):
        from go1_gym_learn.ppo_cse import fused
        t, st = self.transition, self.storage
        s = st.step
        tos = infos['time_outs'] if 'time_outs' in infos else None
        if tos is not None and tos.dtype == torch.bool:
            tos = tos.view(torch.uint8)
        bins = infos["env_bins"][:rewards.shape[0]]
        fused.store_step(self._fused_lib, st, s, rewards.contiguous(), dones if dones.dtype == torch.uint8 else dones.to(torch.uint8), tos,
                         bins if bins.dtype == torch.int32 else bins.to(torch.int32), PPO_Args.gamma)
        st.step += 1
        t.clear()
        self.actor_critic.reset(dones)

    def compute_returns(self, last_critic_obs, last_critic_privileged_obs):
        self.storage.write_history(self._last_hist, last_critic_obs, last_critic_privileged_obs)
        _, last_values = self._infer(self._last_hist)
        self.storage.compute_returns(last_values.clone(), PPO_Args.gamma, PPO_Args.lam,
                                     fused_lib=self._fused_lib if self.fused else None)

    def _adapt_lr(self, kl_mean):
        lr = self._lr
        dk = PPO_Args.desired_kl
        down = torch.clamp(lr / 1.5, min=1e-5)
        up = torch.clamp(lr * 1.5, max=1e-2)
        new = torch.where(kl_mean > dk * 2.0, down, torch.where((kl_mean < dk / 2.0) & (kl_mean > 0.0), up, lr))
        self._lr.copy_(new)
        for group in self.optimizer.param_groups:
            if torch.is_tensor(group['lr']):
                group['lr'].copy_(new)
            else:
                group['lr'] = float(new)

    def _gather(self, idx):
        st = self.storage
        f = lambda t: t.flatten(0, 1)[idx]
        return dict(hist=f(st.observation_histories), priv=f(st.privileged_observations), actions=f(st.actions),
                    values=f(st.values), adv=f(st.advantages), returns=f(st.returns), logp=f(st.actions_log_prob),
                    mu=f(st.mu), sigma=f(st.sigma))

    def _stage_ppo_backward_fused(self, idx):
        net, n = self._train_net, self.n_body
        with torch.no_grad():
            if not self._pregathered:
                self._gather_rows(idx, net.X)
            net.forward(net.X)
            net.ppo_loss(self.storage, idx, self.std, self.master.grad[n:n + self.n_std], PPO_Args, self._kl, self._acc)
            net.backward(net.X)

    def _gather_rows(self, idx, out):
        if self.storage.ring:
            from go1_gym_learn.ppo_cse import fused
            fused.ring_gather(self._fused_lib, self.storage, idx, out)
        else:
            torch.index_select(self.storage.observation_histories.flatten(0, 1), 0, idx, out=out)

    def _stage_adapt_backward_fused(self, idx):
        net = self._train_net
        num_train = int(idx.numel() // 5 * 4)
        with torch.no_grad():
            net.forward_adaptation(net.X)
            net.adaptation_loss(self.storage, idx, num_train, PPO_Args.selective_adaptation_module_loss, self._acc)
            net.backward_adaptation(net.X)

    def _stage_ppo_backward(self, idx):
        if self._train_net is not None:
            return self._stage_ppo_backward_fused(idx)
        A = PPO_Args
        b = self._gather(idx)
        mu_batch, value_batch, _ = self.policy.forward(self.body, b["hist"])
        mu_batch, value_batch = mu_batch.float(), value_batch.float()
        std = self.std
        logp = gaussian_log_prob(b["actions"], mu_batch, std)
        entropy = gaussian_entropy(std)
        with torch.no_grad():
            kl = torch.sum(torch.log(std / b["sigma"] + 1.e-5)
                           + (torch.square(b["sigma"]) + torch.square(b["mu"] - mu_batch)) / (2.0 * torch.square(std)) - 0.5, axis=-1)
            self._kl.copy_(torch.mean(kl))
        ratio = torch.exp(logp - torch.squeeze(b["logp"]))
        adv = torch.squeeze(b["adv"])
        surrogate_loss = torch.max(-adv * ratio, -adv * torch.clamp(ratio, 1.0 - A.clip_param, 1.0 + A.clip_param)).mean()
        if A.use_clipped_value_loss:
            value_clipped = b["values"] + (value_batch - b["values"]).clamp(-A.clip_param, A.clip_param)
            value_loss = torch.max((value_batch - b["returns"]).pow(2), (value_clipped - b["returns"]).pow(2)).mean()
        else:
            value_loss = (b["returns"] - value_batch).pow(2).mean()
        loss = surrogate_loss + A.value_loss_coef * value_loss - A.entropy_coef * entropy
        loss.backward()
        self._pull_grads()
        self._acc[0] += value_loss.detach()
        self._acc[1] += surrogate_loss.detach()

    def _stage_ppo_step(self):
        A = PPO_Args
        sharded = self.dp and self._dp_shard is not None
        if self._opt is not None:
            adaptive = A.desired_kl is not None and A.schedule == 'adaptive'
            w = float(_world()) if self.dp else 1.0
            self._opt.step_(gscale=1.0 / w, max_norm=A.max_grad_norm, kl=self._kl if adaptive else None, kl_scale=1.0 / w,
                            desired_kl=A.desired_kl if adaptive else 0.0, zero_grad=True, zero_slot=self._kl,
                            between=(lambda partial: dist.all_reduce(partial)) if sharded else None,
                            pieces=self._train_net.last_pieces("ppo") if self._train_net is not None else None)
            if sharded:
                self._dp_gather_params()
            return
        g = self._g_live
        if self.dp:
            g.div_(_world())
        if A.desired_kl is not None and A.schedule == 'adaptive':
            self._adapt_lr(self._kl / _world() if self.dp else self._kl)
        self._kl.zero_()
        norm = torch.linalg.vector_norm(g)
        if sharded:
            n2 = norm * norm
            dist.all_reduce(n2)
            norm = n2.sqrt()
        g.mul_(torch.clamp(A.max_grad_norm / (norm + 1e-6), max=1.0))
        self.optimizer.step()
        if sharded:
            self._dp_gather_params()
        else:
            self._push_weights()

    def _stage_adapt_backward(self, idx):
        if self._train_net is not None:
            return self._stage_adapt_backward_fused(idx)
        A = PPO_Args
        st = self.storage
        hist = st.observation_histories.flatten(0, 1)[idx]
        target = st.privileged_observations.flatten(0, 1)[idx]
        num_train = int(target.shape[0] // 5 * 4)
        pred = self.policy.forward(self.body, hist, want_actor=False)[2].float()
        sel = 0 if A.selective_adaptation_module_loss else slice(None)
        adaptation_loss = F.mse_loss(pred[:num_train, sel], target[:num_train, sel])
        with torch.no_grad():
            adaptation_test_loss = F.mse_loss(pred[num_train:, sel], target[num_train:, sel])
        adaptation_loss.backward()
        self._pull_grads()
        self._acc[2] += adaptation_loss.detach()
        self._acc[3] += adaptation_test_loss.detach()

    def _stage_adapt_step(self):
        if self._opt_ad is not None:
            self._opt_ad.step_(gscale=1.0 / float(_world()) if self.dp else 1.0, zero_grad=True,
                               pieces=self._train_net.last_pieces("adaptation") if self._train_net is not None else None)
            return
        if self.dp:
            self.master.grad.div_(_world())
        self.adaptation_module_optimizer.step()
        self._push_weights()

    def _dp_exchange_ppo(self):
        g = self.master.grad
        if self._dp_shard is None:
            if self._dp_lowp is None:
                dist.all_reduce(g)
            else:
                self._dp_lowp.copy_(g)
                dist.all_reduce(self._dp_lowp)
                g.copy_(self._dp_lowp)
            return
        lo, per = self._dp_shard
        self._dp_tail.copy_(g[self.n_body:])
        dist.all_reduce(self._dp_tail)
        src = g
        if self._dp_lowp is not None:
            self._dp_lowp.copy_(g)
            src = self._dp_lowp
        try:
            dist.reduce_scatter_tensor(self._dp_shard_buf, src)
        except (RuntimeError, NotImplementedError):
            dist.all_reduce(src)
            self._dp_shard_buf.copy_(src[lo:lo + per])
        g.zero_()
        g[lo:lo + per].copy_(self._dp_shard_buf)
        self._kl.copy_(self._dp_tail[self.n_std])

    def _dp_gather_params(self):
        lo, per = self._dp_shard
        dist.all_gather_into_tensor(self.master.data, self.master.data[lo:lo + per].clone())
        self._push_weights()

    def _allreduce_adapt_grads(self):
        for v in self._ad_grad_views:
            dist.all_reduce(v)

    def _minibatch_eager(self, idx):
        self._stage_ppo_backward(idx)
        if self.dp:
            self._dp_exchange_ppo()
        self._stage_ppo_step()
        for _ in range(PPO_Args.num_adaptation_module_substeps):
            self._stage_adapt_backward(idx)
            if self.dp:
                self._allreduce_adapt_grads()
            self._stage_adapt_step()

    def _capture(self, i):
        idx = self._idx_all[i]
        single = not self.dp and PPO_Args.num_adaptation_module_substeps == 1
        pool = None
        graphs = []
        if self.dp and PPO_Args.dp_graph_collectives and PPO_Args.num_adaptation_module_substeps == 1 and self._collectives_capturable is not False \
                and dist.get_backend() == "nccl":
            g, err = None, None
            try:
                g = torch.cuda.CUDAGraph()
                with torch.cuda.graph(g, capture_error_mode="thread_local"):
                    self._minibatch_eager(idx)
            except Exception as e:
                g, err = None, e
            ok = torch.tensor([0 if g is None else 1], device=self.device, dtype=torch.int64)
            dist.all_reduce(ok, op=dist.ReduceOp.MIN)
            if int(ok.item()) == 1:
                self._collectives_capturable = True
                return [g]
            if self._collectives_capturable is not False:
                why = f"{type(err).__name__}: {err}" if err is not None else "another rank's capture failed"
                print(f"[ppo] rank {dist.get_rank()}: one-graph capture of stages + collectives not taken ({why}); "
                      f"eager collectives between graphs on every rank", file=sys.stderr)
            self._collectives_capturable = False
            del g
            torch.cuda.synchronize()
            self.master.grad.zero_()

        def rec(fn):
            nonlocal pool
            g = torch.cuda.CUDAGraph()
            with torch.cuda.graph(g, pool=pool, capture_error_mode="thread_local"):
                fn()
            pool = pool or g.pool()
            graphs.append(g)
        if single:
            rec(lambda: self._minibatch_eager(idx))
        else:
            rec(lambda: self._stage_ppo_backward(idx))
            if self._dp_shard is not None:
                rec(lambda: self._stage_adapt_backward(idx))
            else:
                rec(lambda: (self._stage_ppo_step(), self._stage_adapt_backward(idx)))
            rec(self._stage_adapt_step)
        return graphs

    def _minibatch_replay(self, i):
        g = self._graphs[i]
        if len(g) == 1:
            g[0].replay()
            return
        g[0].replay()
        self._dp_exchange_ppo()
        if self._dp_shard is not None:
            self._stage_ppo_step()
        g[1].replay()
        self._allreduce_adapt_grads()
        g[2].replay()

    def update(self):
        A = PPO_Args
        st = self.storage
        batch_size = st.num_envs * st.num_transitions_per_env
        mb = batch_size // A.num_mini_batches
        nmb = A.num_mini_batches
        if self._idx_all is None or tuple(self._idx_all.shape) != (nmb, mb):
            self._idx_all = torch.zeros(nmb, mb, dtype=torch.long, device=self.device)
            self._graphs = {}
            if self.fused:
                from go1_gym_learn.ppo_cse.fused import FusedNet
                self._train_net = FusedNet(self.policy, self.body, self.master.grad[:self.n_body], mb, self._fused_lib, with_grad=True)
                self._train_net.defer_grad_sum = not self.dp
                tr = self._train_net.adam_transposes()
                if tr and self._dp_shard is None:
                    self._train_net.refresh_transposes()
                    self._opt.set_transposes(tr)
                    self._train_net._wt_by_optimizer = True
                self._Xall = torch.zeros(nmb, mb, self.policy.Kp, device=self.device, dtype=self.body.dtype)
        self._acc.zero_()
        if self.fused:
            self.master.grad.zero_()
        indices = torch.randperm(nmb * mb, requires_grad=False, device=self.device)
        self._idx_all.copy_(indices.view(nmb, mb))
        use_graphs = bool(self.on_gpu and A.use_hip_graphs and A.num_adaptation_module_substeps == 1
                          and (self.fused or A.use_hip_graphs == "all"))
        graph_mode = use_graphs and self._updates_done >= 1
        self._pregathered = bool(graph_mode and self.fused)
        if self._pregathered:
            for i in range(nmb):
                self._gather_rows(self._idx_all[i], self._Xall[i])
        if graph_mode and self.fused and not self.dp and self._update_graph_ok and os.environ.get("GO1_UPDATE_GRAPH", "all") == "all":
            key_all = ("all", int(A.num_learning_epochs))
            g = self._graphs.get(key_all)
            if g is None:
                try:
                    g = torch.cuda.CUDAGraph()
                    with torch.cuda.graph(g, capture_error_mode="thread_local"):
                        for epoch in range(A.num_learning_epochs):
                            for i in range(nmb):
                                self._train_net.X = self._Xall[i]
                                self._minibatch_eager(self._idx_all[i])
                    self._graphs[key_all] = g
                except Exception as err:
                    print(f"[ppo] whole-update graph capture failed ({type(err).__name__}: {err}); one graph per mini-batch slot", file=sys.stderr)
                    self._update_graph_ok, g = False, None
                    torch.cuda.synchronize()
                    self.master.grad.zero_()
                    self._acc.zero_()
            if g is not None:
                g.replay()
                return self._finish_update()
        for epoch in range(A.num_learning_epochs):
            for i in range(nmb):
                idx = self._idx_all[i]
                if not self.on_gpu:
                    torch.randn(mb, self.n_std)
                if self.fused:
                    self._train_net.X = self._Xall[i]
                if graph_mode:
                    if i not in self._graphs:
                        try:
                            self._graphs[i] = self._capture(i)
                        except Exception as err:
                            print(f"[ppo] HIP graph capture failed ({type(err).__name__}: {err}); running eagerly", file=sys.stderr)
                            PPO_Args.use_hip_graphs = False
                            graph_mode = self._pregathered = False
                            torch.cuda.synchronize()
                            self.master.grad.zero_()
                            self._minibatch_eager(idx)
                            continue
                    self._minibatch_replay(i)
                else:
                    self._minibatch_eager(idx)
        return self._finish_update()

    def _finish_update(self):
        A = PPO_Args
        self._updates_done += 1
        num_updates = A.num_learning_epochs * A.num_mini_batches
        v, s, a, at = (self._acc / num_updates).tolist()
        a /= A.num_adaptation_module_substeps
        at /= A.num_adaptation_module_substeps
        self.storage.clear()
        return v, s, a, 0.0, 0.0, at, 0.0, 0.0
```

Baseline: 5.068 million.

## Fuse MLP tail forward, PPO/MSE loss, and tail backward into one kernel

Measured after the change: 5.176 million, median of 6. 2.1% higher.

```diff
diff --git a/include/go1ppo.h b/include/go1ppo.h
--- a/include/go1ppo.h
+++ b/include/go1ppo.h
@@ -178,6 +178,33 @@
 } Go1PpoMlp2Bwd;
 int go1ppo_mlp2_bwd(const Go1PpoMlp2Bwd* nets, int count, void* stream);
 
+typedef struct {
+  void* x;
+  const void* W2; const void* b2;
+  const void* W3; const void* b3;
+  void* z2;
+  void* out;
+  void* d_out;
+  void* d_z2;
+  void* d_x;
+  int64_t rows;
+  int32_t ld_x, ld_z2, ld_out, ld_dout, ld_dz2, ld_dx, elu_input, _pad;
+} Go1PpoMlp2Tail;
+
+#define GO1PPO_TAIL_MAX_ACTIONS 12
+int go1ppo_mlp2_tail_ppo(const Go1PpoMlp2Tail* nets, const Go1PpoLossArgs* loss, void* stream);
+
+typedef struct {
+  const float* target;
+  const int64_t* idx;
+  int64_t num_train;
+  int32_t npv, selective;
+  float* d_pred_bias;
+  float* train_loss;
+  float* test_loss;
+} Go1PpoMseArgs;
+int go1ppo_mlp2_tail_mse(const Go1PpoMlp2Tail* net, const Go1PpoMseArgs* mse, void* stream);
+
 const char* go1ppo_version(void);
 
 #ifdef __cplusplus
diff --git a/walk-these-ways_amd/csrc/go1ppo_mlp.h b/walk-these-ways_amd/csrc/go1ppo_mlp.h
--- a/walk-these-ways_amd/csrc/go1ppo_mlp.h
+++ b/walk-these-ways_amd/csrc/go1ppo_mlp.h
@@ -250,6 +250,430 @@
   }
 }
 
+#ifndef MLP2_TAIL_SWZ_RED
+#define MLP2_TAIL_SWZ_RED 0
+#endif
+#define TAIL_AMAX GO1PPO_TAIL_MAX_ACTIONS
+#define DET_TAIL_MAX_TILES (4 * DET_MAX_BLOCKS)
+#define DET_TAIL_PPO_W (4 + 2 * TAIL_AMAX)
+__device__ float det_tail_ppo_slab[DET_TAIL_MAX_TILES * DET_TAIL_PPO_W];
+__device__ float det_tail_mse_slab[DET_TAIL_MAX_TILES * DET_MSE_W];
+__device__ unsigned det_tail_count[2];
+
+struct Mlp2TailPpoArgs { Go1PpoMlp2Tail net[2]; Go1PpoLossArgs loss; };
+struct Mlp2TailMseArgs { Go1PpoMlp2Tail net; Go1PpoMseArgs mse; };
+
+__device__ __forceinline__ int swz_w(int row) { return MLP2_TAIL_SWZ_RED ? swz_red(row) : swz_row(row); }
+__device__ __forceinline__ bf16x8_t lds_tr_operand2(const bf16_t* img, int off_lo, int off_hi) {
+  typedef __attribute__((address_space(3))) s16x4_t lds_s16x4_t;
+  const char* p = reinterpret_cast<const char*>(img);
+  s16x4_t lo = __builtin_amdgcn_ds_read_tr16_b64_v4i16((lds_s16x4_t*)(p + off_lo));
+  s16x4_t hi = __builtin_amdgcn_ds_read_tr16_b64_v4i16((lds_s16x4_t*)(p + off_hi));
+  s16x8_t v = __builtin_shufflevector(lo, hi, 0, 1, 2, 3, 4, 5, 6, 7);
+  return __builtin_bit_cast(bf16x8_t, v);
+}
+#define TAIL_G0 (3 * TAIL_AMAX * 64)
+#define TAIL_MSE_PRE 8
+__device__ __forceinline__ void glds4(const float* g, float* lds_wave_base) {
+  __builtin_amdgcn_global_load_lds((global_cvoid_t*)g, (lds_void_t*)lds_wave_base, 4, 0, 0);
+}
+__device__ __forceinline__ float wave_sum(float x) {
+#pragma unroll
+  for (int o = 32; o > 0; o >>= 1) x += __shfl_xor(x, o, 64);
+  return x;
+}
+
+template <typename F>
+__device__ __forceinline__ void tail_sums(const float* slab, int W, int ncols, int tiles, float* scratch, int floats, F&& publish) {
+  const int groups = (tiles + 3) >> 2, per = floats / ncols;
+  float t = 0.f;
+  for (int b0 = 0; b0 < groups; b0 += per) {
+    const int nb = groups - b0 < per ? groups - b0 : per;
+    for (int i = threadIdx.x; i < nb * ncols; i += MLP2_THREADS) {
+      const int b = b0 + i / ncols, c = i % ncols;
+      float bs = 0.f;
+#pragma unroll
+      for (int q = 0; q < 4; q++) {
+        const int tile = 4 * b + q;
+        bs += tile < tiles ? slab[(int64_t)tile * W + c] : 0.f;
+      }
+      scratch[i] = bs;
+    }
+    __syncthreads();
+    if ((int)threadIdx.x < ncols)
+      for (int i = 0; i < nb; i++) t += scratch[i * ncols + threadIdx.x];
+    __syncthreads();
+  }
+  if ((int)threadIdx.x < ncols) publish((int)threadIdx.x, t);
+}
+
+template <int MODE, int AMAX>
+__device__ __forceinline__ void mlp2_tail_body(const Go1PpoMlp2Tail& N, const Go1PpoLossArgs& L, const Go1PpoMseArgs& Q) {
+  __shared__ __attribute__((aligned(1024))) bf16_t W2i[2 * MLP2_IMG];
+  __shared__ __attribute__((aligned(1024))) bf16_t W3i[64 * 128];
+  __shared__ __attribute__((aligned(1024))) bf16_t Ai[2 * 64 * 128];
+  __shared__ __attribute__((aligned(1024))) bf16_t Z2i[64 * 128];
+  __shared__ __attribute__((aligned(1024))) bf16_t D3i[64 * 128];
+  __shared__ __attribute__((aligned(16))) float Gi[TAIL_G0 + 2 * 64];
+  const int tiles = (int)((N.rows + MLP2_BM - 1) / MLP2_BM);
+  const int t = threadIdx.x, wave = t >> 6, lane = t & 63, r = lane & 15, g = lane >> 4;
+  dma_weights<MLP2_TAIL_SWZ_RED != 0>((const bf16_t*)N.W2, MLP2_N2, MLP2_K1, W2i, wave, lane);
+  dma_weights<MLP2_TAIL_SWZ_RED != 0>((const bf16_t*)N.W3, MLP2_N3, MLP2_N2, W3i, wave, lane);
+  bf16_t* x = (bf16_t*)N.x;
+  bf16_t* z2 = (bf16_t*)N.z2;
+  bf16_t* out = (bf16_t*)N.out;
+  bf16_t* dout = (bf16_t*)N.d_out;
+  bf16_t* dz2 = (bf16_t*)N.d_z2;
+  bf16_t* dx = (bf16_t*)N.d_x;
+  const int tx = g ^ r;
+  int foff[4], woff[4];
+#pragma unroll
+  for (int a = 0; a < 4; a++) {
+    foff[a] = r * 256 + (((4 * a) ^ tx) << 4);
+    woff[a] = r * 256 + (((4 * a + g) ^ swz_w(r)) << 4);
+  }
+  const int nf2 = wave >> 1, mp = (wave & 1) * 2, nf3 = wave & 3, m3 = wave >> 2;
+  float bias2[4], bias3[4];
+  unpack_bf4(*reinterpret_cast<const uint2*>((const bf16_t*)N.b2 + nf2 * 16 + 4 * g), bias2);
+  unpack_bf4(*reinterpret_cast<const uint2*>((const bf16_t*)N.b3 + nf3 * 16 + 4 * g), bias3);
+  const int trow = g * 8 + (r >> 2), tsub = (r & 3) >> 1, thalf = (r & 1) * 8;
+  const int kf2 = wave >> 1;
+  const int w3lo = trow * 256 + (((2 * kf2 + tsub) ^ swz_w(trow)) << 4) + thalf;
+  const int w3hi = (trow + 4) * 256 + (((2 * kf2 + tsub) ^ swz_w(trow + 4)) << 4) + thalf;
+  const bf16_t* w2img = W2i + (wave >> 3) * MLP2_IMG;
+  const int w2lo = trow * 256 + (((2 * (wave & 7) + tsub) ^ swz_w(trow)) << 4) + thalf;
+  const int w2hi = (trow + 4) * 256 + (((2 * (wave & 7) + tsub) ^ swz_w(trow + 4)) << 4) + thalf;
+  const int hch = t & 31;
+  const int zrow = t >> 4, zch = t & 15, drow = (t >> 3) & 63, dch = t & 7;
+  const int zslot = zrow * 256 + ((zch ^ swz_row(zrow)) << 4), dslot = drow * 256 + ((dch ^ swz_row(drow)) << 4);
+  const bool lw = wave == 0;
+  const int lrow = lane * 256, lsw = lane & 15;
+  const bool actor = MODE == 0 && blockIdx.y == 0;
+  const int A = MODE == 0 ? L.num_actions : 0;
+  const bool vec4 = MODE == 0 && (A & 3) == 0 && ((reinterpret_cast<uintptr_t>(L.actions) | reinterpret_cast<uintptr_t>(L.old_mu) |
+                                                  reinterpret_cast<uintptr_t>(L.old_sigma)) & 15) == 0;
+  const int64_t* idx = MODE == 0 ? L.idx : Q.idx;
+  const int ncol = MODE == 1 ? (Q.selective ? 1 : Q.npv) : 0;
+  float* slab = MODE == 0 ? det_tail_ppo_slab : det_tail_mse_slab;
+  const int slabw = MODE == 0 ? DET_TAIL_PPO_W : DET_MSE_W;
+
+  Bf8 v[2];
+  uint4 dv = make_uint4(0, 0, 0, 0);
+  int64_t s = 0;
+  auto fetch = [&](int tile) {
+    const int64_t base = (int64_t)tile * MLP2_BM, last = N.rows - 1;
+#pragma unroll
+    for (int j = 0; j < 2; j++) {
+      const int p = t + MLP2_THREADS * j, row = p >> 5, ch = p & 31;
+      int64_t grow = base + row;
+      grow = grow < N.rows ? grow : last;
+      v[j] = *reinterpret_cast<const Bf8*>(x + grow * N.ld_x + ch * 8);
+    }
+    int64_t q = base + drow;
+    q = q < last ? q : last;
+    if (t < 512) dv = *reinterpret_cast<const uint4*>(dout + q * N.ld_dout + dch * 8);
+    q = base + lane;
+    q = q < last ? q : last;
+    if (lw) s = idx[q];
+  };
+  fetch(blockIdx.x);
+  bool first = true;
+  for (int tile = blockIdx.x; tile < tiles; tile += gridDim.x) {
+    const int64_t row0 = (int64_t)tile * MLP2_BM;
+    const bool on = row0 + lane < N.rows;
+#pragma unroll
+    for (int j = 0; j < 2; j++) {
+      const int p = t + MLP2_THREADS * j, row = p >> 5, ch = p & 31;
+      if (N.elu_input) {
+        float f[8];
+#pragma unroll
+        for (int e = 0; e < 8; e++) f[e] = elu1(bf2f(v[j].v[e]));
+        v[j] = pack_bf8(f);
+        if (row0 + row < N.rows) *reinterpret_cast<Bf8*>(x + (row0 + row) * N.ld_x + ch * 8) = v[j];
+      }
+      *reinterpret_cast<Bf8*>(reinterpret_cast<char*>(Ai + (ch >> 4) * 64 * 128) + row * 256 + (((ch & 15) ^ swz_row(row)) << 4)) = v[j];
+    }
+    if (t < 512) *reinterpret_cast<uint4*>(reinterpret_cast<char*>(D3i) + dslot) = dv;
+    if (lw) {
+      if (MODE == 0 && actor) {
+        if (vec4) {
+#pragma unroll
+          for (int j = 0; j < AMAX; j += 4) {
+            if (j < A) {
+              glds16((const bf16_t*)(L.actions + s * A + j), (bf16_t*)(Gi + (j >> 2) * 256));
+              glds16((const bf16_t*)(L.old_mu + s * A + j), (bf16_t*)(Gi + (3 + (j >> 2)) * 256));
+              glds16((const bf16_t*)(L.old_sigma + s * A + j), (bf16_t*)(Gi + (6 + (j >> 2)) * 256));
+            }
+          }
+        } else {
+#pragma unroll
+          for (int j = 0; j < AMAX; j++) {
+            if (j < A) {
+              glds4(L.actions + s * A + j, Gi + j * 64);
+              glds4(L.old_mu + s * A + j, Gi + (TAIL_AMAX + j) * 64);
+              glds4(L.old_sigma + s * A + j, Gi + (2 * TAIL_AMAX + j) * 64);
+            }
+          }
+        }
+        glds4(L.advantages + s, Gi + TAIL_G0);
+        glds4(L.old_logp + s, Gi + TAIL_G0 + 64);
+      } else if (MODE == 0) {
+        glds4(L.returns + s, Gi + TAIL_G0);
+        if (L.use_clipped_value_loss) glds4(L.old_values + s, Gi + TAIL_G0 + 64);
+      } else {
+#pragma unroll
+        for (int j = 0; j < TAIL_MSE_PRE; j++)
+          if (j < ncol) glds4(Q.target + s * Q.npv + j, Gi + j * 64);
+      }
+    }
+    const int64_t s_cur = s;
+    if (first) asm volatile("s_waitcnt vmcnt(0)" ::: "memory");
+    first = false;
+    __syncthreads();
+    if (tile + (int)gridDim.x < tiles) fetch(tile + gridDim.x);
+    {
+      f32x4 acc[2] = {f32x4{0.f, 0.f, 0.f, 0.f}, f32x4{0.f, 0.f, 0.f, 0.f}};
+#pragma unroll
+      for (int ks = 0; ks < MLP2_K1 / 32; ks++) {
+        const int win = ks >> 2;
+        const bf16x8_t w = lds_b128(W2i + win * MLP2_IMG + nf2 * 16 * 128, woff[ks & 3]);
+#pragma unroll
+        for (int m = 0; m < 2; m++)
+          acc[m] = __builtin_amdgcn_mfma_f32_16x16x32_bf16(w, lds_b128(Ai + win * 64 * 128 + (mp + m) * 16 * 128, foff[ks & 3]), acc[m], 0, 0, 0);
+      }
+      const int n0 = nf2 * 16 + 4 * g;
+#pragma unroll
+      for (int m = 0; m < 2; m++) {
+        const int row = (mp + m) * 16 + r;
+        float o4[4];
+#pragma unroll
+        for (int e = 0; e < 4; e++) o4[e] = elu1(acc[m][e] + bias2[e]);
+        const uint2 o = pack_bf4(o4);
+        if (row0 + row < N.rows) *reinterpret_cast<uint2*>(z2 + (row0 + row) * N.ld_z2 + n0) = o;
+        *reinterpret_cast<uint2*>(reinterpret_cast<char*>(Z2i) + row * 256 + (((n0 >> 3) ^ swz_row(row)) << 4) + ((n0 >> 2) & 1) * 8) = o;
+      }
+    }
+    __syncthreads();
+    {
+      f32x4 acc = f32x4{0.f, 0.f, 0.f, 0.f};
+#pragma unroll
+      for (int ks = 0; ks < MLP2_N2 / 32; ks++)
+        acc = __builtin_amdgcn_mfma_f32_16x16x32_bf16(lds_b128(W3i + nf3 * 16 * 128, woff[ks]), lds_b128(Z2i + m3 * 16 * 128, foff[ks]), acc, 0, 0, 0);
+      const int n0 = nf3 * 16 + 4 * g, row = m3 * 16 + r;
+      float o4[4];
+#pragma unroll
+      for (int e = 0; e < 4; e++) o4[e] = acc[e] + bias3[e];
+      const uint2 o = pack_bf4(o4);
+      if (row0 + row < N.rows) *reinterpret_cast<uint2*>(out + (row0 + row) * N.ld_out + n0) = o;
+      *reinterpret_cast<uint2*>(reinterpret_cast<char*>(D3i) + row * 256 + ((((n0 >> 3) | 8) ^ swz_row(row)) << 4) + ((n0 >> 2) & 1) * 8) = o;
+    }
+    if (lw) asm volatile("s_waitcnt vmcnt(0)" ::: "memory");
+    __syncthreads();
+    auto gat = [&](int which, int j) -> float& { return vec4 ? Gi[(which * 3 + (j >> 2)) * 256 + lane * 4 + (j & 3)] : Gi[(which * TAIL_AMAX + j) * 64 + lane]; };
+    if (MODE == 0 && actor) {
+#pragma clang fp contract(off)
+      const Go1PpoLossArgs& a = L;
+      char* d3 = reinterpret_cast<char*>(D3i) + lrow;
+      float* prow = slab + (int64_t)tile * slabw;
+      const float invM = 1.f / (float)a.rows;
+      const float HALF_LOG_2PI = 0.9189385332046727f;
+      const int j = wave;
+      if (j < A) {
+        const float mu = bf2f(*reinterpret_cast<const bf16_t*>(d3 + ((((j >> 3) | 8) ^ lsw) << 4) + (j & 7) * 2));
+        float sg = a.std[j];
+        float isg = 1.f / sg;
+        const float zj = (gat(0, j) - mu) * isg;
+        float so = gat(2, j), dm = gat(1, j) - mu;
+        gat(0, j) = zj;
+        gat(1, j) = fmaf(-0.5f * zj, zj, -logf(sg)) - HALF_LOG_2PI;
+        gat(2, j) = logf(sg / so + 1.e-5f) + fmaf(dm, dm, so * so) / (2.f * sg * sg) - 0.5f;
+      }
+      __syncthreads();
+      if (lw) {
+        float logp = 0.f, kl = 0.f;
+        for (int q = 0; q < A; q++) {
+          logp += gat(1, q);
+          kl += gat(2, q);
+        }
+        float adv = Gi[TAIL_G0 + lane];
+        float ratio = expf(logp - Gi[TAIL_G0 + 64 + lane]);
+        float lo = 1.f - a.clip_param, hi = 1.f + a.clip_param;
+        float rc = fminf(fmaxf(ratio, lo), hi);
+        float s1 = -adv * ratio, s2 = -adv * rc;
+        float sur = fmaxf(s1, s2) * invM;
+        float dratio = (ratio >= lo && ratio <= hi) ? -adv : (s1 > s2 ? -adv : 0.f);
+        float dlogp = dratio * ratio * invM;
+        kl *= invM;
+        Gi[TAIL_G0 + lane] = dlogp;
+        sur = wave_sum(on ? sur : 0.f);
+        kl = wave_sum(on ? kl : 0.f);
+        if (lane == 0) { det_put(prow, sur); det_put(prow + 2, kl); }
+      }
+      __syncthreads();
+      if (j < A) {
+        const float dlogp = Gi[TAIL_G0 + lane];
+        const float isg = 1.f / a.std[j], zj = gat(0, j);
+        const bf16_t gq = f2bf(dlogp * zj * isg);
+        if (on) *reinterpret_cast<bf16_t*>(d3 + (((j >> 3) ^ lsw) << 4) + (j & 7) * 2) = gq;
+        float dmb = bf2f(gq);
+        float dstd = dlogp * fmaf(zj, zj, -1.f) * isg;
+        dstd = wave_sum(on ? dstd : 0.f);
+        dmb = wave_sum(on ? dmb : 0.f);
+        if (lane == 0) { det_put(prow + 4 + j, dstd); det_put(prow + 4 + TAIL_AMAX + j, dmb); }
+      }
+    } else if (lw) {
+#pragma clang fp contract(off)
+      char* d3 = reinterpret_cast<char*>(D3i) + lrow;
+      const int64_t rr = row0 + lane;
+      float* prow = slab + (int64_t)tile * slabw;
+      const float g0 = Gi[TAIL_G0 + lane], g1 = Gi[TAIL_G0 + 64 + lane];
+      if (MODE == 0) {
+        const Go1PpoLossArgs& a = L;
+        const float invM = 1.f / (float)a.rows;
+        float vl = 0.f, dvb = 0.f;
+        if (on) {
+          float v = bf2f(*reinterpret_cast<const bf16_t*>(d3 + ((8 ^ lsw) << 4)));
+          float R = g0, dval;
+          if (a.use_clipped_value_loss) {
+            float vo = g1;
+            float dlt = v - vo;
+            float vc = vo + fminf(fmaxf(dlt, -a.clip_param), a.clip_param);
+            float l1 = (v - R) * (v - R), l2 = (vc - R) * (vc - R);
+            vl = fmaxf(l1, l2) * invM;
+            bool inside = dlt >= -a.clip_param && dlt <= a.clip_param;
+            dval = inside ? 2.f * (v - R) : (l1 > l2 ? 2.f * (v - R) : 0.f);
+          } else {
+            vl = (R - v) * (R - v) * invM;
+            dval = 2.f * (v - R);
+          }
+          bf16_t gv = f2bf(a.value_loss_coef * dval * invM);
+          dout[rr * N.ld_dout] = gv;
+          *reinterpret_cast<bf16_t*>(d3 + (lsw << 4)) = gv;
+          dvb = bf2f(gv);
+        }
+        vl = wave_sum(vl);
+        dvb = wave_sum(dvb);
+        if (lane == 0) { det_put(prow + 1, vl); det_put(prow + 3, dvb); }
+      } else {
+        const int npv = Q.npv;
+        const int64_t rows = N.rows, num_train = Q.num_train;
+        float ltrain = 0.f, ltest = 0.f;
+        float inv_train = 1.f / ((float)num_train * ncol), inv_test = 1.f / ((float)(rows - num_train) * ncol);
+        bf16_t* d_pred = dout + rr * N.ld_dout;
+        for (int j = 0; j < ncol; j++) {
+          float vj = 0.f;
+          if (on) {
+            const float tj = j < TAIL_MSE_PRE ? Gi[j * 64 + lane] : Q.target[s_cur * npv + j];
+            float e = bf2f(*reinterpret_cast<const bf16_t*>(d3 + ((((j >> 3) | 8) ^ lsw) << 4) + (j & 7) * 2)) - tj;
+            bf16_t gj = 0;
+            if (rr < num_train) {
+              ltrain = fmaf(e * e, inv_train, ltrain);
+              gj = f2bf(2.f * e * inv_train);
+              vj = bf2f(gj);
+            } else {
+              ltest = fmaf(e * e, inv_test, ltest);
+            }
+            d_pred[j] = gj;
+            *reinterpret_cast<bf16_t*>(d3 + (((j >> 3) ^ lsw) << 4) + (j & 7) * 2) = gj;
+          }
+          vj = wave_sum(vj);
+          if (lane == 0) det_put(prow + j, vj);
+        }
+        ltrain = wave_sum(ltrain);
+        ltest = wave_sum(ltest);
+        if (lane == 0) { det_put(prow + ncol, ltrain); det_put(prow + ncol + 1, ltest); }
+        if (Q.selective && on)
+          for (int j = 1; j < npv; j++) {
+            d_pred[j] = 0;
+            *reinterpret_cast<bf16_t*>(d3 + (((j >> 3) ^ lsw) << 4) + (j & 7) * 2) = 0;
+          }
+      }
+    }
+    __syncthreads();
+    if (MODE == 0 && actor && t < 512 && row0 + drow < N.rows)
+      *reinterpret_cast<uint4*>(dout + (row0 + drow) * N.ld_dout + dch * 8) = *reinterpret_cast<const uint4*>(reinterpret_cast<const char*>(D3i) + dslot);
+    {
+      f32x4 acc[2] = {f32x4{0.f, 0.f, 0.f, 0.f}, f32x4{0.f, 0.f, 0.f, 0.f}};
+#pragma unroll
+      for (int kk = 0; kk < MLP2_N3 / 32; kk++) {
+        const bf16x8_t w = lds_tr_operand2(W3i, kk * 32 * 256 + w3lo, kk * 32 * 256 + w3hi);
+#pragma unroll
+        for (int m = 0; m < 2; m++) acc[m] = __builtin_amdgcn_mfma_f32_16x16x32_bf16(w, lds_b128(D3i + (mp + m) * 16 * 128, foff[kk]), acc[m], 0, 0, 0);
+      }
+      const int k0 = kf2 * 16 + 4 * g;
+#pragma unroll
+      for (int m = 0; m < 2; m++) {
+        const int row = (mp + m) * 16 + r;
+        uint2* slot = reinterpret_cast<uint2*>(reinterpret_cast<char*>(Z2i) + row * 256 + (((k0 >> 3) ^ swz_row(row)) << 4) + ((k0 >> 2) & 1) * 8);
+        float h[4], o4[4];
+        unpack_bf4(*slot, h);
+#pragma unroll
+        for (int e = 0; e < 4; e++) o4[e] = acc[m][e] * (h[e] > 0.f ? 1.f : h[e] + 1.f);
+        *slot = pack_bf4(o4);
+      }
+    }
+    __syncthreads();
+    {
+      f32x4 acc[4];
+#pragma unroll
+      for (int m = 0; m < 4; m++) acc[m] = f32x4{0.f, 0.f, 0.f, 0.f};
+#pragma unroll
+      for (int kk = 0; kk < MLP2_N2 / 32; kk++) {
+        const bf16x8_t w = lds_tr_operand2(w2img, kk * 32 * 256 + w2lo, kk * 32 * 256 + w2hi);
+#pragma unroll
+        for (int m = 0; m < 4; m++) acc[m] = __builtin_amdgcn_mfma_f32_16x16x32_bf16(w, lds_b128(Z2i + m * 16 * 128, foff[kk]), acc[m], 0, 0, 0);
+      }
+      const int k0 = (wave & 7) * 16 + 4 * g;
+#pragma unroll
+      for (int m = 0; m < 4; m++) {
+        const int row = m * 16 + r;
+        uint2* slot = reinterpret_cast<uint2*>(reinterpret_cast<char*>(Ai + (wave >> 3) * 64 * 128) + row * 256 +
+                                               (((k0 >> 3) ^ swz_row(row)) << 4) + ((k0 >> 2) & 1) * 8);
+        float h[4], o4[4];
+        unpack_bf4(*slot, h);
+#pragma unroll
+        for (int e = 0; e < 4; e++) o4[e] = acc[m][e] * (h[e] > 0.f ? 1.f : h[e] + 1.f);
+        *slot = pack_bf4(o4);
+      }
+    }
+    __syncthreads();
+    if (row0 + zrow < N.rows) put16_wt(dz2 + (row0 + zrow) * N.ld_dz2 + zch * 8, *reinterpret_cast<const uint4*>(reinterpret_cast<const char*>(Z2i) + zslot));
+#pragma unroll
+    for (int j = 0; j < 2; j++)
+      if (row0 + MLP2_HROW(j) < N.rows)
+        put16_wt(dx + (row0 + MLP2_HROW(j)) * N.ld_dx + hch * 8, *reinterpret_cast<const uint4*>(reinterpret_cast<const char*>(Ai) + MLP2_HSLOT(j)));
+    __syncthreads();
+  }
+  if (!det_last(&det_tail_count[MODE], gridDim.x * gridDim.y)) return;
+  float* scratch = reinterpret_cast<float*>(Ai);
+  if (MODE == 0) {
+    const Go1PpoLossArgs& a = L;
+    tail_sums(slab, slabw, DET_TAIL_PPO_W, tiles, scratch, 2 * 64 * 128 / 2, [&](int c, float tsum) {
+      const int j = c < 4 ? 0 : (c - 4) % TAIL_AMAX;
+      if (c >= 4 && j >= A) return;
+      float* dst = c < 4 ? (c == 0 ? a.surrogate_loss : c == 1 ? a.value_loss : c == 2 ? a.kl : a.d_value_bias)
+                         : c < 4 + TAIL_AMAX ? a.d_std + j : a.d_mean_bias + j;
+      if (!dst) return;
+      float sres = *dst + tsum;
+      if (c >= 4 && c < 4 + TAIL_AMAX) sres += -a.entropy_coef / a.std[j];
+      *dst = sres;
+    });
+  } else {
+    tail_sums(slab, slabw, ncol + 2, tiles, scratch, 2 * 64 * 128 / 2, [&](int c, float tsum) {
+      float* dst = c < ncol ? (Q.d_pred_bias ? Q.d_pred_bias + c : nullptr) : c == ncol ? Q.train_loss : Q.test_loss;
+      if (dst) *dst += tsum;
+    });
+  }
+}
+
+template <int AMAX>
+__global__ __launch_bounds__(MLP2_THREADS, 1) void mlp2_tail_ppo_kernel(Mlp2TailPpoArgs A) {
+  mlp2_tail_body<0, AMAX>(A.net[blockIdx.y], A.loss, Go1PpoMseArgs{});
+}
+__global__ __launch_bounds__(MLP2_THREADS, 1) void mlp2_tail_mse_kernel(Mlp2TailMseArgs A) {
+  mlp2_tail_body<1, 4>(A.net, Go1PpoLossArgs{}, A.mse);
+}
+
 static inline bool aligned8(const void* p) { return (reinterpret_cast<uintptr_t>(p) & 7) == 0; }
 
 extern "C" int go1ppo_mlp2_fwd(const Go1PpoMlp2Fwd* nets, int count, void* stream) {
@@ -290,3 +714,59 @@
   mlp2_bwd_kernel<<<dim3((unsigned)wgs, count), dim3(MLP2_THREADS), 0, (hipStream_t)stream>>>(A);
   return hipGetLastError() == hipSuccess ? 0 : -9;
 }
+
+static int mlp2_tail_check(const Go1PpoMlp2Tail& N) {
+  if (!N.x || !N.W2 || !N.b2 || !N.W3 || !N.b3 || !N.z2 || !N.out || !N.d_out || !N.d_z2 || !N.d_x || N.rows <= 0) return -1;
+  if ((N.rows + MLP2_BM - 1) / MLP2_BM > DET_TAIL_MAX_TILES) return -1;
+  return 0;
+}
+static int mlp2_tail_check_shape(const Go1PpoMlp2Tail& N) {
+  if ((N.ld_x & 7) || (N.ld_z2 & 7) || (N.ld_dz2 & 7) || (N.ld_dx & 7) || N.ld_x < MLP2_K1 || N.ld_z2 < MLP2_N2 || N.ld_dz2 < MLP2_N2 ||
+      N.ld_dx < MLP2_K1 || N.ld_out != MLP2_N3 || N.ld_dout != MLP2_N3 || !aligned16(N.x) || !aligned16(N.W2) || !aligned16(N.W3) ||
+      !aligned8(N.b2) || !aligned8(N.b3) || !aligned16(N.z2) || !aligned16(N.out) || !aligned16(N.d_out) || !aligned16(N.d_z2) ||
+      !aligned16(N.d_x) || N.d_z2 == N.z2 || N.d_x == N.x)
+    return -2;
+  return 0;
+}
+
+extern "C" int go1ppo_mlp2_tail_ppo(const Go1PpoMlp2Tail* nets, const Go1PpoLossArgs* loss, void* stream) {
+  if (!nets || !loss) return -1;
+  for (int i = 0; i < 2; i++)
+    if (mlp2_tail_check(nets[i])) return -1;
+  const Go1PpoLossArgs& a = *loss;
+  if (!a.std || !a.idx || !a.actions || !a.old_mu || !a.old_sigma || !a.old_logp || !a.advantages || !a.returns ||
+      (a.use_clipped_value_loss && !a.old_values) || a.rows <= 0 || a.num_actions <= 0 || a.num_actions > GO1PPO_TAIL_MAX_ACTIONS)
+    return -1;
+  for (int i = 0; i < 2; i++)
+    if (mlp2_tail_check_shape(nets[i])) return -2;
+  if (a.head_ld != MLP2_N3 || a.rows != nets[0].rows || a.rows != nets[1].rows || a.mean != nets[0].out || a.value != nets[1].out ||
+      a.d_mean != nets[0].d_out || a.d_value != nets[1].d_out)
+    return -2;
+  Mlp2TailPpoArgs A;
+  A.net[0] = nets[0];
+  A.net[1] = nets[1];
+  A.loss = a;
+  int64_t wgs = (a.rows + MLP2_BM - 1) / MLP2_BM;
+  if (wgs > 128) wgs = 128;
+  const dim3 grid((unsigned)wgs, 2), block(MLP2_THREADS);
+  if (a.num_actions <= 4) mlp2_tail_ppo_kernel<4><<<grid, block, 0, (hipStream_t)stream>>>(A);
+  else if (a.num_actions <= 8) mlp2_tail_ppo_kernel<8><<<grid, block, 0, (hipStream_t)stream>>>(A);
+  else mlp2_tail_ppo_kernel<12><<<grid, block, 0, (hipStream_t)stream>>>(A);
+  return hipGetLastError() == hipSuccess ? 0 : -9;
+}
+
+extern "C" int go1ppo_mlp2_tail_mse(const Go1PpoMlp2Tail* net, const Go1PpoMseArgs* mse, void* stream) {
+  if (!net || !mse) return -1;
+  if (mlp2_tail_check(*net)) return -1;
+  if (!mse->target || !mse->idx || !mse->train_loss || !mse->test_loss || mse->num_train <= 0 || mse->num_train >= net->rows || mse->npv <= 0 ||
+      mse->npv > GO1PPO_HEAD)
+    return -1;
+  if (mlp2_tail_check_shape(*net)) return -2;
+  Mlp2TailMseArgs A;
+  A.net = *net;
+  A.mse = *mse;
+  int64_t wgs = (net->rows + MLP2_BM - 1) / MLP2_BM;
+  if (wgs > 256) wgs = 256;
+  mlp2_tail_mse_kernel<<<dim3((unsigned)wgs), dim3(MLP2_THREADS), 0, (hipStream_t)stream>>>(A);
+  return hipGetLastError() == hipSuccess ? 0 : -9;
+}
diff --git a/walk-these-ways_amd/go1_gym_learn/ppo_cse/fused.py b/walk-these-ways_amd/go1_gym_learn/ppo_cse/fused.py
--- a/walk-these-ways_amd/go1_gym_learn/ppo_cse/fused.py
+++ b/walk-these-ways_amd/go1_gym_learn/ppo_cse/fused.py
@@ -66,7 +66,18 @@
                [(n, ctypes.c_int32) for n in ("ld_dout", "ld_z2", "ld_h", "ld_dz2", "ld_dx", "_pad")]
 
 
+class Mlp2Tail(ctypes.Structure):
+    _fields_ = [(n, ctypes.c_void_p) for n in ("x", "W2", "b2", "W3", "b3", "z2", "out", "d_out", "d_z2", "d_x")] + [("rows", ctypes.c_int64)] + \
+               [(n, ctypes.c_int32) for n in ("ld_x", "ld_z2", "ld_out", "ld_dout", "ld_dz2", "ld_dx", "elu_input", "_pad")]
+
+
+class MseArgs(ctypes.Structure):
+    _fields_ = [("target", ctypes.c_void_p), ("idx", ctypes.c_void_p), ("num_train", ctypes.c_int64), ("npv", ctypes.c_int32),
+                ("selective", ctypes.c_int32), ("d_pred_bias", ctypes.c_void_p), ("train_loss", ctypes.c_void_p), ("test_loss", ctypes.c_void_p)]
+
+
 MLP2_DIMS = (256, 128, 64)
+TAIL_MAX_ACTIONS = 12
 
 
 class GemmArgs(ctypes.Structure):
@@ -83,7 +94,7 @@
     _fields_ = [("num_transposes", ctypes.c_int32), ("_pad", ctypes.c_int32), ("transpose", _AdamTranspose * 2)]
 
 
-EXPORTED_SYMBOLS = ["go1ppo_mlp2_fwd", "go1ppo_mlp2_bwd", "go1ppo_gemm_nt", "go1ppo_gemm_nt_pair", "go1ppo_sum_partials", "go1ppo_wgrad_tn_plan", "go1ppo_wgrad_tn_batched", "go1ppo_tail_fwd", "go1ppo_elu_fwd", "go1ppo_elu_bwd", "go1ppo_loss", "go1ppo_mse", "go1ppo_wgrad", "go1ppo_wgrad_plan",
+EXPORTED_SYMBOLS = ["go1ppo_mlp2_fwd", "go1ppo_mlp2_bwd", "go1ppo_mlp2_tail_ppo", "go1ppo_mlp2_tail_mse", "go1ppo_gemm_nt", "go1ppo_gemm_nt_pair", "go1ppo_sum_partials", "go1ppo_wgrad_tn_plan", "go1ppo_wgrad_tn_batched", "go1ppo_tail_fwd", "go1ppo_elu_fwd", "go1ppo_elu_bwd", "go1ppo_loss", "go1ppo_mse", "go1ppo_wgrad", "go1ppo_wgrad_plan",
                     "go1ppo_wgrad_batched", "go1ppo_act",
                     "go1ppo_store_step", "go1ppo_ring_snapshot", "go1ppo_ring_step", "go1ppo_ring_gather", "go1ppo_gae", "go1ppo_normalize", "go1ppo_opt_partials", "go1ppo_opt_prestep",
                     "go1ppo_opt_prestep_pieces", "go1ppo_grad_reduce", "go1ppo_opt_adam", "go1ppo_version"]
@@ -111,6 +122,8 @@
     L.go1ppo_sum_partials.argtypes = [vp, i32, i64, i64, i32, vp, i32, i32, i32, vp]
     L.go1ppo_mlp2_fwd.argtypes = [ctypes.POINTER(Mlp2Fwd), i32, vp]
     L.go1ppo_mlp2_bwd.argtypes = [ctypes.POINTER(Mlp2Bwd), i32, vp]
+    L.go1ppo_mlp2_tail_ppo.argtypes = [ctypes.POINTER(Mlp2Tail), ctypes.POINTER(LossArgs), vp]
+    L.go1ppo_mlp2_tail_mse.argtypes = [ctypes.POINTER(Mlp2Tail), ctypes.POINTER(MseArgs), vp]
     L.go1ppo_wgrad_batched.argtypes = [vp, i32, i32, vp]
     L.go1ppo_wgrad_tn_plan.argtypes = [ctypes.POINTER(WgradProblem), i32]
     L.go1ppo_wgrad_tn_batched.argtypes = [vp, i32, i32, vp]
@@ -221,6 +234,7 @@
                           and tuple(self.P[f"{n}.{self.depth[n] - 1}.W"].shape) == (MLP2_DIMS[2], MLP2_DIMS[1]) for n in self.depth)
                       and self.depth["adaptation"] == 3 and self.depth["actor"] == 4 and self.depth["critic"] == 4)
         self._mlp2_cache = {}
+        self._tail_in_loss = False
         na1, nc1 = int(self.P["actor.1.W"].shape[0]), int(self.P["critic.1.W"].shape[0])
         nt_ok = all(v % 64 == 0 for v in (na1, nc1, self.na, self.n1 - self.nd - self.na)) and \
             all(self.P[k].data_ptr() % 16 == 0 for k in ("actor.1.b", "critic.1.b", "actor.1.W", "critic.1.W"))
@@ -351,6 +365,39 @@
         arr, n = self._mlp2_cache[key]
         _chk(self.lib.go1ppo_mlp2_bwd(arr, n, _stream()), "go1ppo_mlp2_bwd")
 
+    def _mlp2_tail(self, key, items):
+        key = ("tail", key)
+        if key not in self._mlp2_cache:
+            arr = (Mlp2Tail * len(items))()
+            for a, (net, x, d_x) in zip(arr, items):
+                d = self.depth[net]
+                W2, W3, z2, out = self.P[f"{net}.{d - 2}.W"], self.P[f"{net}.{d - 1}.W"], self.Z[net][d - 2], self.Z[net][d - 1]
+                d_out, d_z2 = self.dZ[net][d - 1], self.dZ[net][d - 2]
+                a.x, a.W2, a.b2, a.W3, a.b3 = x.data_ptr(), W2.data_ptr(), self.P[f"{net}.{d - 2}.b"].data_ptr(), W3.data_ptr(), self.P[f"{net}.{d - 1}.b"].data_ptr()
+                a.z2, a.out, a.d_out, a.d_z2, a.d_x, a.rows = z2.data_ptr(), out.data_ptr(), d_out.data_ptr(), d_z2.data_ptr(), d_x.data_ptr(), x.shape[0]
+                a.ld_x, a.ld_z2, a.ld_out, a.ld_dout, a.ld_dz2, a.ld_dx, a.elu_input = _ld(x), _ld(z2), _ld(out), _ld(d_out), _ld(d_z2), _ld(d_x), 1
+            self._mlp2_cache[key] = arr
+        return self._mlp2_cache[key]
+
+    def _tail_ok(self, arr):
+        for a in arr:
+            if a.ld_out != HEAD or a.ld_dout != HEAD or a.ld_x % 8 or a.ld_z2 % 8 or a.ld_dz2 % 8 or a.ld_dx % 8 or a.d_x == a.x or a.d_z2 == a.z2:
+                return False
+            if any(p % 16 for p in (a.x, a.W2, a.W3, a.z2, a.out, a.d_out, a.d_z2, a.d_x)) or a.b2 % 8 or a.b3 % 8:
+                return False
+        return True
+
+    def tail_ppo_fused(self, num_actions):
+        if not (self._mlp2 and self.G is not None and 0 < num_actions <= TAIL_MAX_ACTIONS):
+            return False
+        Z, dZ = self.Z, self.dZ
+        return self._tail_ok(self._mlp2_tail("ac", [("actor", Z["actor"][1], dZ["actor"][1]), ("critic", Z["critic"][1], dZ["critic"][1])]))
+
+    def tail_adaptation_fused(self):
+        if not (self._mlp2 and self.G is not None):
+            return False
+        return self._tail_ok(self._mlp2_tail("adaptation_only", [("adaptation", self.Y1d, self.dH1["adaptation"])]))
+
     def _forward_mlp2(self, x):
         P, Z, nd, na = self.P, self.Z, self.nd, self.na
         torch.mm(x, P["W1"].t(), out=self.Y1)
@@ -369,14 +416,16 @@
                 torch.addmm(P["critic.1.b"], self.Y1[:, nd + na:], P["critic.1.W"].t(), out=Z["critic"][1])
             torch.addmm(P["actor.1.b"], self.Y1[:, nd:nd + na], P["actor.1.W"].t(), out=Z["actor"][1])
         self._join()
-        self._mlp2_fwd("ac", [("actor", Z["actor"][1]), ("critic", Z["critic"][1])])
+        if not self._tail_in_loss:
+            self._mlp2_fwd("ac", [("actor", Z["actor"][1]), ("critic", Z["critic"][1])])
         return Z["actor"][3], Z["critic"][3], latent
 
     def _backward_mlp2(self, x):
         nd, na = self.nd, self.na
         P, G, Z, dZ, Y1, dY1, dH1 = self.P, self.G, self.Z, self.dZ, self.Y1, self.dY1, self.dH1
         cols = {"adaptation": slice(0, nd), "actor": slice(nd, nd + na), "critic": slice(nd + na, self.n1)}
-        self._mlp2_bwd("ac", [("actor", Z["actor"][1], dZ["actor"][1]), ("critic", Z["critic"][1], dZ["critic"][1])])
+        if not self._tail_in_loss:
+            self._mlp2_bwd("ac", [("actor", Z["actor"][1], dZ["actor"][1]), ("critic", Z["critic"][1], dZ["critic"][1])])
         for net in ("actor", "critic"):
             self._wgrad(dZ[net][3], Z[net][2], G[f"{net}.3.W"], None)
             self._wgrad(dZ[net][2], Z[net][1], G[f"{net}.2.W"], G[f"{net}.2.b"])
@@ -410,12 +459,14 @@
 
     def _forward_adaptation_mlp2(self, x):
         torch.mm(x, self.P["W1"][:self.nd].t(), out=self.Y1d)
-        self._mlp2_fwd("adaptation_only", [("adaptation", self.Y1d)])
+        if not self._tail_in_loss:
+            self._mlp2_fwd("adaptation_only", [("adaptation", self.Y1d)])
         return self.Z["adaptation"][2]
 
     def _backward_adaptation_mlp2(self, x):
         nd, d, G, Z, dZ = self.nd, self.dH1["adaptation"], self.G, self.Z, self.dZ
-        self._mlp2_bwd("adaptation_only", [("adaptation", self.Y1d, d)])
+        if not self._tail_in_loss:
+            self._mlp2_bwd("adaptation_only", [("adaptation", self.Y1d, d)])
         self._wgrad(dZ["adaptation"][2], Z["adaptation"][1], G["adaptation.2.W"], None)
         self._wgrad(dZ["adaptation"][1], self.Y1d, G["adaptation.1.W"], G["adaptation.1.b"])
         self._big_wgrad(d, x, G["W1"][:nd], self._w1_tmp[:, :nd], own_kernel=self._wgrad_tn)
@@ -609,6 +660,11 @@
         a.kl = kl.data_ptr()
         a.value_loss = acc[0:].data_ptr()
         a.surrogate_loss = acc[1:].data_ptr()
+        if self._tail_in_loss:
+            Z, dZ = self.Z, self.dZ
+            arr = self._mlp2_tail("ac", [("actor", Z["actor"][1], dZ["actor"][1]), ("critic", Z["critic"][1], dZ["critic"][1])])
+            _chk(self.lib.go1ppo_mlp2_tail_ppo(arr, ctypes.byref(a), _stream()), "go1ppo_mlp2_tail_ppo")
+            return
         _chk(self.lib.go1ppo_loss(ctypes.byref(a), _stream()), "go1ppo_loss")
 
     def adaptation_loss(self, st, idx, num_train, selective, acc):
@@ -616,6 +672,13 @@
         pred, dpred = self.Z["adaptation"][last], self.dZ["adaptation"][last]
         target = st.privileged_observations.flatten(0, 1)
         assert target.is_contiguous() and target.dtype == torch.float32 and target.shape[1] == self.pol.npv
+        if self._tail_in_loss:
+            arr = self._mlp2_tail("adaptation_only", [("adaptation", self.Y1d, self.dH1["adaptation"])])
+            q = MseArgs()
+            q.target, q.idx, q.num_train, q.npv, q.selective = target.data_ptr(), idx.data_ptr(), num_train, self.pol.npv, int(selective)
+            q.d_pred_bias, q.train_loss, q.test_loss = self.G[f"adaptation.{last}.b"].data_ptr(), acc[2:].data_ptr(), acc[3:].data_ptr()
+            _chk(self.lib.go1ppo_mlp2_tail_mse(arr, ctypes.byref(q), _stream()), "go1ppo_mlp2_tail_mse")
+            return
         _chk(self.lib.go1ppo_mse(pred.data_ptr(), HEAD, target.data_ptr(), self.pol.npv, idx.data_ptr(), self.M, num_train,
                                  int(selective), dpred.data_ptr(), self.G[f"adaptation.{last}.b"].data_ptr(),
                                  acc[2:].data_ptr(), acc[3:].data_ptr(), _stream()), "go1ppo_mse")
diff --git a/walk-these-ways_amd/go1_gym_learn/ppo_cse/ppo.py b/walk-these-ways_amd/go1_gym_learn/ppo_cse/ppo.py
--- a/walk-these-ways_amd/go1_gym_learn/ppo_cse/ppo.py
+++ b/walk-these-ways_amd/go1_gym_learn/ppo_cse/ppo.py
@@ -359,9 +359,13 @@
         with torch.no_grad():
             if not self._pregathered:
                 self._gather_rows(idx, net.X)
-            net.forward(net.X)
-            net.ppo_loss(self.storage, idx, self.std, self.master.grad[n:n + self.n_std], PPO_Args, self._kl, self._acc)
-            net.backward(net.X)
+            net._tail_in_loss = net.tail_ppo_fused(self.std.numel())
+            try:
+                net.forward(net.X)
+                net.ppo_loss(self.storage, idx, self.std, self.master.grad[n:n + self.n_std], PPO_Args, self._kl, self._acc)
+                net.backward(net.X)
+            finally:
+                net._tail_in_loss = False
 
     def _gather_rows(self, idx, out):
         if self.storage.ring:
@@ -374,9 +378,13 @@
         net = self._train_net
         num_train = int(idx.numel() // 5 * 4)
         with torch.no_grad():
-            net.forward_adaptation(net.X)
-            net.adaptation_loss(self.storage, idx, num_train, PPO_Args.selective_adaptation_module_loss, self._acc)
-            net.backward_adaptation(net.X)
+            net._tail_in_loss = net.tail_adaptation_fused()
+            try:
+                net.forward_adaptation(net.X)
+                net.adaptation_loss(self.storage, idx, num_train, PPO_Args.selective_adaptation_module_loss, self._acc)
+                net.backward_adaptation(net.X)
+            finally:
+                net._tail_in_loss = False
 
     def _stage_ppo_backward(self, idx):
         if self._train_net is not None:
```
